# tabahi/WebSpeechAnalyzer

Measured on AMD Instinct MI355X. Metric: 53-feat frames/sec, higher is better.
Workload: dtype f32 front end / f64 tracker; 1 GPU; 1024 clips x 10 s @16 kHz mono per GPU, 1024-pt FFT, 25 ms hop, Segment Features (level 5); parallelism=1 GPU, batches_in_flight=6, streams=3

## Files before the change

webspeechanalyzer_amd/capi.py:

```python
import ctypes
import os
import subprocess

import numpy as np

_HERE = os.path.dirname(os.path.abspath(__file__))
NFEAT = 53


class WsaError(RuntimeError):
    pass


class _Config(ctypes.Structure):
    _fields_ = [("spec_type", ctypes.c_int32), ("output_level", ctypes.c_int32),
                ("f_min", ctypes.c_double), ("f_max", ctypes.c_double),
                ("N_fft_bins", ctypes.c_int32), ("N_mel_bins", ctypes.c_int32),
                ("window_width", ctypes.c_double), ("window_step", ctypes.c_double),
                ("pause_length", ctypes.c_double), ("min_seg_length", ctypes.c_double),
                ("auto_noise_gate", ctypes.c_int32),
                ("voiced_max_dB", ctypes.c_double), ("voiced_min_dB", ctypes.c_double),
                ("pre_norm_gain", ctypes.c_double), ("high_f_emph", ctypes.c_double)]


# ... 426 lines not shown
        return CHANNEL_MIX
    if isinstance(select, (bool, float)) or not 0 <= int(select) <= CHANNEL_MIX:
        raise WsaError(f"select {select!r}: a channel index or 'mix'")
    s = int(select)
    if channels is not None and s != CHANNEL_MIX and s >= int(channels):
        raise WsaError(f"select {s} is neither a channel below {int(channels)} nor 'mix'")
    return s


def pcm_decode(fmt, array, channels=1, select=0):
    f = pcm_format(fmt)
    ch = int(channels)
    if not 1 <= ch <= 64:
        raise WsaError(f"channel count {ch} outside 1 .. 64")
    sel = channel_select(select, ch)
    a = _pcm_array(fmt, f, array)
    size = a.size // _PCM_ELEMS.get(f, 1)
    last = ch - 1 if sel == CHANNEL_MIX else sel
    n = (size - 1 - last) // ch + 1 if size > last else 0
    out = np.zeros(n, np.float32)
    if lib().wsa_pcm_decode_select(f, a.ctypes.data, n, ch, sel, out.ctypes.data) != 0:
        raise WsaError("wsa_pcm_decode_select refused its arguments")
    return out


def pcm_channels_tile_frames(fmt, channels):
    return int(lib().wsa_pcm_channels_tile_frames(pcm_format(fmt), int(channels)))


def level_feature_count(output_level):
    return int(lib().wsa_level_feature_count(int(output_level)))


def rows_to_callbacks(level, step, meta, feat, payload):
    cbs = []
    if level in (4, 5):
        for m, f in zip(meta, feat):
            cbs.append([int(m[1]), [], [m[2] * step, (m[3] + 1) * step], payload(m, f)])
    elif level in (10, 12, 13):
        i = 0
        while i < len(meta):
            j = i
            while j < len(meta) and meta[j][1] == meta[i][1]:
                j += 1
            tm = [["%.3f" % (m[2] * step), "%.3f" % ((m[3] + 1) * step)] for m in meta[i:j]]
            rows_ = list(zip(meta[i:j], feat[i:j]))
            if level == 12:
                cut = next((q for q, (_, f) in enumerate(rows_) if f[23] != 0), len(rows_))
                rows_ = rows_[:cut]
            if level != 12 or rows_:
                cbs.append([int(meta[i][1]), [], tm, [payload(m, f) for m, f in rows_]])
            i = j
    return cbs


class Config(dict):

    def __init__(self, **kw):
        c = _Config()
        lib().wsa_config_default(ctypes.byref(c))
        super().__init__({k: getattr(c, k) for k, _ in _Config._fields_})
        for k, v in kw.items():
            if k not in self:
                raise KeyError(k)
            self[k] = v

    def c_struct(self):
        c = _Config()
        for k, t in _Config._fields_:
            setattr(c, k, int(self[k]) if t is ctypes.c_int32 else float(self[k]))
        return c


class Analyzer:

    def __init__(self, config=None, device=0):
        self.L = lib()
        self.config = config or Config()
        self.h = ctypes.c_void_p()
        cs = self.config.c_struct()
        st = self.L.wsa_create(ctypes.byref(cs), device, ctypes.byref(self.h))
        if st != 0:
            raise WsaError(f"wsa_create failed ({st}): {self.L.wsa_last_error(None).decode()}")
        self.device = device

    def _check(self, st):
        if st != 0:
            raise WsaError(f"libwsa error {st}: {self.L.wsa_last_error(self.h).decode()}")

    def geometry(self, fs):
        g = _Geometry()
        self._check(self.L.wsa_geometry_for(self.h, float(fs), ctypes.byref(g)))
        return {k: getattr(g, k) for k, _ in _Geometry._fields_}

    def bins_hz(self, fs):
        n = self.geometry(fs)["bands"]
        out = np.zeros(n)
        self._check(self.L.wsa_bins_hz(self.h, float(fs), out.ctypes.data, n))
        return out

    def batch(self, n_samples, fs, resample_to=None):
        return Batch(self, n_samples, fs, resample_to)

    def streams(self, n_streams, fs, frames_per_step=1, max_span_frames=1024, resample_to=None):
        return Streams(self, n_streams, fs, frames_per_step, max_span_frames, resample_to)

    def load_model(self, src):
        from . import nnmodel
        if isinstance(src, nnmodel.ModelSpec):
            spec = src
        elif isinstance(src, (tuple, list)):
            spec = nnmodel.parse(*src)
        else:
            spec = nnmodel.load_dir(src)
        return Model(self, spec)

    def trainer(self, spec, features, labels, n_val, batch_size, learning_rate):
        return Trainer(self, spec, features, labels, n_val, batch_size, learning_rate)

    def regress_trainer(self, spec, features, values, n_val, batch_size, learning_rate, out_min=None, out_max=None):
        return Trainer(self, spec, features, values, n_val, batch_size, learning_rate,
                       regression=(spec.out_min if out_min is None else out_min, spec.out_max if out_max is None else out_max))

    def train_group(self, trainers):
        return TrainGroup(self, trainers)

    def feature_db(self, features, durations, vocab_sizes=(), n_ord=0, first_row=0):
        return FeatureDBStats(self, features, durations, vocab_sizes, n_ord, first_row)

    def device_db(self, width, capacity):
        return FeatDB(self, width, capacity)

    def knn_store(self, width, n_classes, capacity):
        return KnnStore(self, width, n_classes, capacity)

    def ensemble(self, models):
        return Ensemble(self, models)

    def regress_group(self, models, ranges=None):
        return RegressGroup(self, models, ranges)

    def close(self):
        if self.h:
            self.L.wsa_destroy(self.h)
            self.h = ctypes.c_void_p()

    def __del__(self):
        try:
            self.close()
        except Exception:
            pass


class Batch:

    def __init__(self, an, n_samples, fs, resample_to=None):
        self.an, self.L = an, an.L
        self.n_samples = np.ascontiguousarray(n_samples, dtype=np.uint32)
        self.fs = float(fs) if np.ndim(fs) == 0 else None
        self.h = ctypes.c_void_p()
        if self.fs is None and not resample_to:
            raise WsaError("one rate per clip needs resample_to: a launch has one geometry")
        if resample_to and np.ndim(fs) > 0:
            self.n_samples_in, self.fs_in, self.fs = self.n_samples, np.ascontiguousarray(fs, dtype=np.float64), float(resample_to)
            if self.fs_in.shape != self.n_samples_in.shape:
                raise WsaError("fs as a sequence holds one rate per clip")
            an._check(self.L.wsa_batch_create_mixed(an.h, len(self.n_samples_in), self.n_samples_in.ctypes.data, self.fs_in.ctypes.data, self.fs, ctypes.byref(self.h)))
            self.n_samples = np.array([self.L.wsa_resample_length(int(n), float(f), self.fs) for n, f in zip(self.n_samples_in, self.fs_in)], np.uint32)
        elif resample_to:
            self.n_samples_in, self.fs_in, self.fs = self.n_samples, self.fs, float(resample_to)
            an._check(self.L.wsa_batch_create_resampled(an.h, len(self.n_samples_in), self.n_samples_in.ctypes.data, self.fs_in, self.fs, ctypes.byref(self.h)))
            self.n_samples = np.array([self.L.wsa_resample_length(int(n), self.fs_in, self.fs) for n in self.n_samples_in], np.uint32)
        else:
            an._check(self.L.wsa_batch_create(an.h, len(self.n_samples), self.n_samples.ctypes.data, self.fs, ctypes.byref(self.h)))
        info = _BatchInfo()
        an._check(self.L.wsa_batch_get_info(self.h, ctypes.byref(info)))
        self.info = {k: getattr(info, k) for k, _ in _BatchInfo._fields_}

    def run(self, d_pcm, clip_stride, stream=0):
        self.an._check(self.L.wsa_batch_run(self.h, d_pcm, int(clip_stride), stream))

    def run_frontend(self, d_pcm, clip_stride, stream=0):
        self.an._check(self.L.wsa_batch_run_frontend(self.h, d_pcm, int(clip_stride), stream))

    def run_backend(self, d_spectra, stream=0):
        self.an._check(self.L.wsa_batch_run_backend(self.h, d_spectra, stream))

    def converted_pcm(self, stream=0):
        stride = max(int(self.n_samples.max()) if len(self.n_samples) else 0, 1)
        out = np.zeros((len(self.n_samples), stride), np.float32)
        self.an._check(self.L.wsa_batch_copy_pcm(self.h, stream, out.ctypes.data, stride))
        return out

    def run_host(self, clips, stream=0):
        clips = [np.ascontiguousarray(c, dtype=np.float32) for c in clips]
        ptrs = (ctypes.c_void_p * len(clips))(*[c.ctypes.data for c in clips])
        self.an._check(self.L.wsa_batch_run_host(self.h, ptrs, stream))

    def run_host_i16(self, clips, channels=None, stream=0):
        clips = [np.ascontiguousarray(c, dtype=np.int16) for c in clips]
        ptrs = (ctypes.c_void_p * len(clips))(*[c.ctypes.data for c in clips])
        ch = None if channels is None else (ctypes.c_uint32 * len(clips))(*[int(c) for c in channels])
        self.an._check(self.L.wsa_batch_run_host_i16(self.h, ptrs, ch, stream))

    def _formats(self, formats, channels):
        n = len(self.n_samples)
        fm = [formats] * n if isinstance(formats, (str, int)) else list(formats)
        if len(fm) != n or (channels is not None and len(channels) != n):
            raise WsaError("one format (and one channel count) per clip")
        fm = (ctypes.c_int32 * max(n, 1))(*[pcm_format(f) if isinstance(f, str) else int(f) for f in fm])
        ch = None if channels is None else (ctypes.c_uint32 * max(n, 1))(*[int(c) for c in channels])
        return fm, ch

    def run_host_packed(self, clips, formats, channels=None, stream=0):
        fm, ch = self._formats(formats, channels)
        held = []
        ns_in = getattr(self, "n_samples_in", self.n_samples)
        for i, c in enumerate(clips):
            f = int(fm[i])
            a = _pcm_array(f, f, c) if f in _PCM_DTYPE else np.ascontiguousarray(c).reshape(-1)
            need = int(ns_in[i]) * (int(ch[i]) if ch is not None else 1) * _PCM_ELEMS.get(f, 1)
            if f in _PCM_DTYPE and a.size < need:
                raise WsaError(f"clip {i}: {a.size} elements, the plan's {int(ns_in[i])} frames need {need}")
            held.append(a)
        ptrs = (ctypes.c_void_p * max(len(held), 1))(*[a.ctypes.data for a in held])
        self.an._check(self.L.wsa_batch_run_host_packed(self.h, ptrs, fm, ch, stream))

    def set_input_format(self, formats, channels=None):
        fm, ch = self._formats(formats, channels)
        self.an._check(self.L.wsa_batch_set_input_format(self.h, fm, ch))

    def packed_offsets(self):
        return np.array([self.L.wsa_batch_packed_offset(self.h, i) for i in range(len(self.n_samples) + 1)], np.uint64)

    def run_packed(self, d_packed, stream=0):
        self.an._check(self.L.wsa_batch_run_packed(self.h, d_packed, stream))

    def _select_source(self, select, source):
        n = len(self.n_samples)
        sel = None
        if select is not None:
            sv = [select] * n if isinstance(select, (str, int)) else list(select)
            if len(sv) != n:
                raise WsaError("one select (a channel index or 'mix') per clip")
            sel = (ctypes.c_uint32 * max(n, 1))(*[channel_select(v) for v in sv])
        src = None
        if source is not None:
            if len(source) != n:
                raise WsaError("one source (a clip index) per clip")
            if any(int(v) < 0 or int(v) > 0xFFFFFFFF for v in source):
                raise WsaError("a source is a clip index")
            src = (ctypes.c_uint32 * max(n, 1))(*[int(v) for v in source])
        return sel, src

    def set_input_channels(self, formats, channels=None, select=None, source=None):
        fm, ch = self._formats(formats, channels)
        sel, src = self._select_source(select, source)
        self.an._check(self.L.wsa_batch_set_input_channels(self.h, fm, ch, sel, src))

    def run_host_channels(self, clips, formats, channels=None, select=None, source=None, stream=0):
        fm, ch = self._formats(formats, channels)
        sel, src = self._select_source(select, source)
        held, ptrs = [], []
        ns_in = getattr(self, "n_samples_in", self.n_samples)
        for i, c in enumerate(clips):
            if src is not None and int(src[i]) != i:
                ptrs.append(None)
                continue
            f = int(fm[i])
            a = _pcm_array(f, f, c) if f in _PCM_DTYPE else np.ascontiguousarray(c).reshape(-1)
            need = int(ns_in[i]) * (int(ch[i]) if ch is not None else 1) * _PCM_ELEMS.get(f, 1)
            if f in _PCM_DTYPE and a.size < need:
                raise WsaError(f"clip {i}: {a.size} elements, the plan's {int(ns_in[i])} frames need {need}")
            held.append(a)
            ptrs.append(a.ctypes.data)
        if len(ptrs) != len(self.n_samples):
            raise WsaError("one entry per clip (a consumer's may be None)")
        arr = (ctypes.c_void_p * max(len(ptrs), 1))(*ptrs)
        self.an._check(self.L.wsa_batch_run_host_channels(self.h, arr, fm, ch, sel, src, stream))

    def enable_timing(self, on):
        self.an._check(self.L.wsa_batch_enable_timing(self.h, int(on)))

    def keep_spectra(self, on=True):
        self.an._check(self.L.wsa_batch_keep_spectra(self.h, int(on)))
        return self

    def backend_reruns(self):
        n = ctypes.c_uint32(0)
        self.an._check(self.L.wsa_batch_backend_reruns(self.h, ctypes.byref(n)))
        return n.value

    def keep_counters(self, on=True):
        self.L.wsa_debug_batch_keep_counters.argtypes = [ctypes.c_void_p, ctypes.c_int32]
        self.an._check(self.L.wsa_debug_batch_keep_counters(self.h, int(on)))
        return self

    def tiers(self, stream=0):
        out = (ctypes.c_uint32 * 3)()
        self.L.wsa_debug_batch_tiers.argtypes = [ctypes.c_void_p, ctypes.c_void_p, ctypes.c_void_p]
        self.an._check(self.L.wsa_debug_batch_tiers(self.h, stream, out))
        return dict(flags=int(out[0]), spans=int(out[1]), redo=int(out[2]))

    def enable_trace(self, on=True):
        self.an._check(self.L.wsa_batch_enable_trace(self.h, int(on)))

    def trace(self, stream=0):
        n = self.info["n_frames_total"]
        out = np.zeros((n, 12))
        self.an._check(self.L.wsa_batch_copy_trace(self.h, stream, out.ctypes.data, max(n, 1)))
        return out

    def device_result(self, stream=0):
        r = _DeviceResult()
        self.an._check(self.L.wsa_batch_result(self.h, stream, ctypes.byref(r)))
        return r

    def stage_ms(self):
        out = np.zeros(4, np.float32)
        self.an._check(self.L.wsa_batch_stage_ms(self.h, out.ctypes.data))
        return out

    def rows(self, stream=0):
        r = self.device_result(stream)
        n, m, nc = r.n_rows, r.n_segments, r.n_clips
        meta = np.zeros((n, 8), np.int32)
        feat = np.zeros((n, NFEAT), np.float64)
        segs = np.zeros((m, 4), np.int32)
        roff = np.zeros(nc + 1, np.uint32)
        soff = np.zeros(nc + 1, np.uint32)
        self.an._check(self.L.wsa_batch_copy_rows(self.h, stream, meta.ctypes.data, feat.ctypes.data, max(n, 1),
                                                   segs.ctypes.data, max(m, 1), roff.ctypes.data, soff.ctypes.data))
        return dict(meta=meta, feat=feat, segments=segs, row_off=roff, seg_off=soff)

    def row_meta(self, stream=0):
        n = self.device_result(stream).n_rows
        meta = np.zeros((n, 8), np.int32)
        self.an._check(self.L.wsa_batch_copy_rows(self.h, stream, meta.ctypes.data, None, max(n, 1), None, 0, None, None))
        return meta

    def utterance_meta(self, stream=0):
        n = self.device_result(stream).n_utterance_rows
        meta = np.zeros((n, 4), np.int32)
        self.an._check(self.L.wsa_batch_copy_utterance(self.h, stream, meta.ctypes.data, None, max(n, 1), None))
        return meta

    def spectra(self, stream=0):
        words = self.info["n_frames_total"] * self.info["bands"]
        out = np.zeros((self.info["n_frames_total"], self.info["bands"]), np.uint32)
        foff = np.zeros(self.info["n_clips"] + 1, np.uint32)
        self.an._check(self.L.wsa_batch_copy_spectra(self.h, stream, out.ctypes.data, max(words, 1), foff.ctypes.data))
        return out, foff

    def formants(self, stream=0):
        n = self.info["n_frames_total"]
        out = np.zeros((n, 9), np.float32)
        self.an._check(self.L.wsa_batch_copy_formants(self.h, stream, out.ctypes.data, max(n, 1)))
        return out

    def utterance(self, stream=0):
        r = self.device_result(stream)
        n = r.n_utterance_rows
        meta = np.zeros((n, 4), np.int32)
        feat = np.zeros((n, 264), np.float64)
        off = np.zeros(len(self.n_samples) + 1, np.uint32)
        self.an._check(self.L.wsa_batch_copy_utterance(self.h, stream, meta.ctypes.data, feat.ctypes.data, max(n, 1), off.ctypes.data))
        return dict(meta=meta, feat=feat, off=off)

    def tracks(self, stream=0):
        class _TI(ctypes.Structure):
            _fields_ = [("n_segments", ctypes.c_uint32), ("n_points", ctypes.c_uint64), ("n_ranked", ctypes.c_uint64)]
        ti = _TI()
        self.an._check(self.L.wsa_batch_tracks_info(self.h, stream, ctypes.byref(ti)))
        seg_off = np.zeros((ti.n_segments + 1, 2), np.uint64)
        pts = np.zeros((max(int(ti.n_points), 1), 8), np.int32)
        rk = np.zeros(max(int(ti.n_ranked), 1), np.int32)
        self.an._check(self.L.wsa_batch_copy_tracks(self.h, stream, seg_off.ctypes.data, pts.ctypes.data, int(ti.n_points), rk.ctypes.data, int(ti.n_ranked)))
        return _track_records(seg_off, pts, rk, ti.n_segments)

    def callbacks(self, stream=0):
        r = self.rows(stream)
        level = int(self.an.config["output_level"])
        step = float(self.an.config["window_step"]) / 1e3
        utt = self.utterance(stream) if level == 11 else None
        trk = self.tracks(stream) if level == 3 else None
        fm = self.formants(stream) if level in (4, 10) else None
        foff = None
        if fm is not None:
            foff = np.zeros(len(self.n_samples) + 1, np.uint32)
            self.an._check(self.L.wsa_batch_copy_spectra(self.h, stream, None, 0, foff.ctypes.data))
        out = []
        for c in range(len(self.n_samples)):
            a, b = int(r["row_off"][c]), int(r["row_off"][c + 1])
            meta, feat = r["meta"][a:b], r["feat"][a:b]
            cbs = []
            payload = (lambda m, f: f[:23].copy() if level == 12 else f.copy()) if fm is None else (lambda m, f: fm[int(foff[c]) + m[6]: int(foff[c]) + m[6] + m[7]].copy())
            if level == 11:
                for k in range(int(utt["off"][c]), int(utt["off"][c + 1])):
                    m = utt["meta"][k]
                    cbs.append([0, [], [m[2] * step, (m[3] + 1) * step], utt["feat"][k].copy()])
            else:
                cbs = rows_to_callbacks(level, step, meta, feat, payload)
            sa, sb = int(r["seg_off"][c]), int(r["seg_off"][c + 1])
            if level == 3:
                cbs = [[k, [], trk[sa + k]] for k in range(sb - sa) if len(trk[sa + k]) > 0]
            out.append(dict(callbacks=cbs, segments_ci=[[int(s[1]), int(s[2])] for s in r["segments"][sa:sb]],
                            flags=[int(s[3]) for s in r["segments"][sa:sb]], meta=meta))
        return out

    def classify(self, model, stream=0):
        self.an._check(self.L.wsa_batch_classify(self.h, model.h, stream))
        self._model = model

    def class_result(self, stream=0):
        r = _ClassResult()
        self.an._check(self.L.wsa_batch_class_result(self.h, stream, ctypes.byref(r)))
        return r

    def classes(self, stream=0):
        r = self.class_result(stream)
        C, n, k = int(r.n_classes), int(r.n_rows), int(r.n_callbacks)
        prob, cb = np.zeros((n, C), np.float32), np.zeros((k, 4), np.int32)
        lab, conf = np.zeros(k, np.int32), np.zeros(k, np.float64)
        clip = np.zeros((int(r.n_clips), C), np.float64) if r.d_clip_conf else np.zeros((0, C))
        self.an._check(self.L.wsa_batch_copy_classes(self.h, stream, prob.ctypes.data, max(n, 1), cb.ctypes.data, lab.ctypes.data, conf.ctypes.data,
                                                      max(k, 1), clip.ctypes.data if r.d_clip_conf else None))
        return dict(prob=prob, cb=cb, cb_label=lab, cb_conf=conf, clip_conf=clip, labels=list(self._model.labels))

    def regress(self, model, out_min=None, out_max=None, stream=0):
        lo, hi = model.out_range(out_min, out_max)
        self.an._check(self.L.wsa_batch_regress(self.h, model.h, lo, hi, stream))
        self._model = model

    def values(self, stream=0):
        n = ctypes.c_uint32()
        self.an._check(self.L.wsa_batch_copy_values(self.h, stream, None, 0, ctypes.byref(n)))
        out = np.zeros(n.value, np.float64)
        self.an._check(self.L.wsa_batch_copy_values(self.h, stream, out.ctypes.data, max(n.value, 1), ctypes.byref(n)))
        return out

    def knn(self, store, k=10, stream=0):
        self.an._check(self.L.wsa_batch_knn(self.h, store.h, int(k), stream))
        self._knn = store

    def knn_result(self, stream=0):
        r = _KnnResult()
        self.an._check(self.L.wsa_batch_knn_result(self.h, stream, ctypes.byref(r)))
        return r

    def knn_classes(self, stream=0):
        r = self.knn_result(stream)
        n, C, k = int(r.n_rows), int(r.n_classes), int(r.k)
        out = dict(label=np.zeros(n, np.int32), conf=np.zeros((n, C), np.float64), nbr=np.zeros((n, k), np.int32), sim=np.zeros((n, k), np.float32), k_eff=int(r.k_eff))
        self.an._check(self.L.wsa_batch_copy_knn(self.h, stream, out["label"].ctypes.data, out["conf"].ctypes.data, out["nbr"].ctypes.data, out["sim"].ctypes.data, max(n, 1)))
        return out

    def knn_fold(self, stream=0):
        self.an._check(self.L.wsa_batch_knn_fold(self.h, stream))

    def knn_fold_classes(self, stream=0):
        r = _KnnFoldResult()
        self.an._check(self.L.wsa_batch_knn_fold_result(self.h, stream, ctypes.byref(r)))
        k, C = int(r.n_callbacks), int(r.n_classes)
        out = dict(cb=np.zeros((k, 4), np.int32), cb_label=np.zeros(k, np.int32), cb_conf=np.zeros(k, np.float64), clip_conf=np.zeros((int(r.n_clips), C), np.float64))
        self.an._check(self.L.wsa_batch_copy_knn_fold(self.h, stream, out["cb"].ctypes.data, out["cb_label"].ctypes.data, out["cb_conf"].ctypes.data, max(k, 1),
                                                       out["clip_conf"].ctypes.data))
        return out

    def regress_group(self, group, stream=0):
        self.an._check(self.L.wsa_batch_regress_group(self.h, group.h, stream))
        self._group = group

    def value_result(self, stream=0):
        r = _ValueResult()
        self.an._check(self.L.wsa_batch_value_result(self.h, stream, ctypes.byref(r)))
        return r

    def value_fold(self, stream=0):
        r = self.value_result(stream)
        H, n, k, nc = int(r.n_heads), int(r.n_rows), int(r.n_callbacks), int(r.n_clips)
        out = dict(value=np.zeros((H, n), np.float64))
        if r.d_cb:
            out.update(cb=np.zeros((k, 4), np.int32), cb_value=np.zeros((H, k)), cb_weight=np.zeros((H, k)),
                       clip_sum=np.zeros((H, nc)), clip_weight=np.zeros((H, nc)), clip_value=np.zeros((H, nc)))
        h = _ValueHost()
        h.rows_cap, h.cb_cap = max(n, 1), max(k, 1)
        for name, v in out.items():
            if name == "cb":
                h.cb = v.ctypes.data
            else:
                for d in range(H):
                    getattr(h, name)[d] = v[d].ctypes.data
        self.an._check(self.L.wsa_batch_copy_value_fold(self.h, stream, ctypes.byref(h)))
        return out

    def classify_ensemble(self, ensemble, stream=0):
        self.an._check(self.L.wsa_batch_classify_ensemble(self.h, ensemble.h, stream))
        self._ensemble = ensemble

    def ensemble_result(self, stream=0):
        r = _EnsembleResult()
        self.an._check(self.L.wsa_batch_ensemble_result(self.h, stream, ctypes.byref(r)))
        return r

    def ensemble_classes(self, stream=0):
        r = self.ensemble_result(stream)
        nm, n, k, nc = int(r.n_members), int(r.n_rows), int(r.n_callbacks), int(r.n_clips)
        fold = bool(r.d_cb)
        C = [int(r.n_classes[d]) for d in range(nm)]
        out = dict(prob=[np.zeros((n, c), np.float32) for c in C], labels=[list(m.labels) for m in self._ensemble.models])
        h = _EnsembleHost()
        h.rows_cap, h.cb_cap = max(n, 1), max(k, 1)
        if fold:
            for name, dt in (("cb_label", np.int32), ("cb_conf", np.float64), ("cb_all_max", np.float64)):
                out[name] = [np.zeros(k, dt) for _ in C]
            out["clip_conf"] = [np.zeros((nc, c), np.float64) for c in C]
            out.update(cb=np.zeros((k, 4), np.int32), cb_db=np.zeros(k, np.int32), cb_top_label=np.zeros(k, np.int32), cb_top_conf=np.zeros(k),
                       cb_min_db=np.zeros(k, np.int32), cb_entropy=np.zeros(k), clip_min_db=np.zeros(nc, np.int32))
        for name, v in out.items():
            if name == "labels":
                continue
            if isinstance(v, list):
                for d in range(nm):
                    getattr(h, name)[d] = v[d].ctypes.data
            else:
                setattr(h, name, v.ctypes.data)
        self.an._check(self.L.wsa_batch_copy_ensemble(self.h, stream, ctypes.byref(h)))
        return out

    def close(self):
        if self.h:
            self.L.wsa_batch_destroy(self.h)
            self.h = ctypes.c_void_p()

    def __del__(self):
        try:
            self.close()
        except Exception:
            pass


def _model_desc(spec):
    from . import nnmodel
    nl = len(spec.kernels)
    keep = [np.ascontiguousarray(k, np.float32) for k in spec.kernels] + [np.ascontiguousarray(b, np.float32) for b in spec.biases]
    units = (ctypes.c_int32 * (nl + 1))(*spec.units)
    acts = (ctypes.c_int32 * nl)(*[nnmodel.ACT[a] for a in spec.activations])
    kp = (ctypes.c_void_p * nl)(*[a.ctypes.data for a in keep[:nl]])
    bp = (ctypes.c_void_p * nl)(*[a.ctypes.data for a in keep[nl:]])
    mn, mx = np.ascontiguousarray(spec.in_min, np.float64), np.ascontiguousarray(spec.in_max, np.float64)
    labels = list(spec.labels)
    lab = (ctypes.c_char_p * len(labels))(*[str(x).encode() for x in labels]) if len(labels) == spec.n_classes else None
    d = _ModelDesc(nl, ctypes.cast(units, ctypes.c_void_p), ctypes.cast(acts, ctypes.c_void_p), ctypes.cast(kp, ctypes.c_void_p),
                   ctypes.cast(bp, ctypes.c_void_p), mn.ctypes.data, mx.ctypes.data, ctypes.cast(lab, ctypes.c_void_p) if lab is not None else None)
    return d, (keep, units, acts, kp, bp, mn, mx, lab)


class Model:

    def __init__(self, an, spec):
        self.an, self.L, self.spec = an, an.L, spec
        self.labels = list(spec.labels)
        self.n_classes = spec.n_classes
        self.n_inputs = int(spec.units[0])
        d, self._keep = _model_desc(spec)
        self.h = ctypes.c_void_p()
        an._check(self.L.wsa_model_create(an.h, ctypes.byref(d), ctypes.byref(self.h)))
        self._keep = None

    def classify_rows(self, d_feat, n_rows, d_prob, stream=0):
        self.an._check(self.L.wsa_classify_rows(self.h, d_feat, int(n_rows), d_prob, stream))

    def out_range(self, out_min=None, out_max=None):
        lo = getattr(self.spec, "out_min", None) if out_min is None else out_min
        hi = getattr(self.spec, "out_max", None) if out_max is None else out_max
        if lo is None or hi is None:
            raise ValueError("the model has no output range (out_min / out_max): not a regression model's spec, and none was given")
        return float(lo), float(hi)

    def regress_rows(self, d_feat, n_rows, d_value, out_min=None, out_max=None, stream=0):
        lo, hi = self.out_range(out_min, out_max)
        self.an._check(self.L.wsa_regress_rows(self.h, lo, hi, d_feat, int(n_rows), d_value, stream))

    def close(self):
        if self.h:
            self.L.wsa_model_destroy(self.h)
            self.h = ctypes.c_void_p()

    def __del__(self):
        try:
            self.close()
        except Exception:
            pass


class Trainer:

    def __init__(self, an, spec, features, labels, n_val, batch_size, learning_rate, regression=None, db=None):
        self.an, self.L, self.spec = an, an.L, spec
        self.out_range = None if regression is None else (float(regression[0]), float(regression[1]))
        lab = np.ascontiguousarray(labels, np.int32 if regression is None else np.float64)
        if db is not None:
            rows = np.ascontiguousarray(features, np.uint32)
            if rows.ndim != 1 or lab.shape != rows.shape:
                raise ValueError(f"rows {rows.shape} / labels {lab.shape}: expected [n] DB row indices and [n]")
            self.n_rows, self.n_val, self.n_train = rows.shape[0], int(n_val), rows.shape[0] - int(n_val)
# ... 1172 lines not shown
```

webspeechanalyzer_amd/csrc/api.hip:

```cpp
#include <cstdlib>
#include <map>
#include <mutex>
#include "host_plan.hpp"
#include "pcm_formats.hpp"

using namespace wsa;

thread_local std::string wsa_api::g_create_error;
using wsa_api::fail;

namespace wsa {
Tuning Tuning::from_env() {
    Tuning t;
    { const char* on = std::getenv("WSA_TUNING_ENV"); if (!on || on[0] != '1') return t; }
    auto num = [](const char* name, int dflt) { const char* e = std::getenv(name); return e && *e ? std::atoi(e) : dflt; };
    t.dbg = num("WSA_DBG", 0);
    t.no_pair = std::getenv("WSA_NO_PAIR") != nullptr; t.no_split = std::getenv("WSA_NO_SPLIT") != nullptr; t.no_quad = std::getenv("WSA_NO_QUAD") != nullptr; t.quad = std::getenv("WSA_QUAD") != nullptr; t.no_fuse = std::getenv("WSA_NO_FUSE") != nullptr;
    t.fe_fat = std::getenv("WSA_FE_FAT") != nullptr; t.peaks_lanes = std::getenv("WSA_PEAKS_LANES") != nullptr;
    t.full_table = num("WSA_FULL_TABLE", -1);
    t.tracker_wpc = num("WSA_TRACKER_WPC", 0); t.fin_wpc = num("WSA_FIN_WPC", 0); t.fpw = num("WSA_FPW", 0);
    t.fe_wg_per_cu = num("WSA_FE_WGS", 0); t.fe_no_queue = std::getenv("WSA_FE_NO_QUEUE") != nullptr; t.peaks_wpc = num("WSA_PEAKS_WPC", 0); t.peaks_w = num("WSA_PEAKS_W", 0); t.upload_threads = num("WSA_UPLOAD_THREADS", 0);
    t.rs_s = num("WSA_RS_S", 0); t.rs_j = num("WSA_RS_J", 0); t.rs_c = num("WSA_RS_C", 0); t.rs_one_launch = std::getenv("WSA_RS_ONE_LAUNCH") != nullptr;
    return t;
}
}

static std::mutex g_slab_mu;
static std::map<uintptr_t, size_t> g_slabs;
bool wsa_api::slab_of(const void* p, uintptr_t* base, size_t* size) {
    std::lock_guard<std::mutex> lk(g_slab_mu);
    auto it = g_slabs.upper_bound(reinterpret_cast<uintptr_t>(p));
    if (it == g_slabs.begin()) return false;
    --it;
    if (reinterpret_cast<uintptr_t>(p) >= it->first + it->second) return false;
    *base = it->first; *size = it->second;
    return true;
}

extern "C" {

int wsa_abi_version(void) { return WSA_ABI_VERSION; }

void wsa_config_default(wsa_config* c) {
    c->spec_type = 1; c->output_level = 4; c->f_min = 50; c->f_max = 4000; c->N_fft_bins = 256; c->N_mel_bins = 128;
    c->window_width = 25; c->window_step = 25; c->pause_length = 200; c->min_seg_length = 50; c->auto_noise_gate = 1;
    c->voiced_max_dB = 100; c->voiced_min_dB = 10; c->pre_norm_gain = 1000; c->high_f_emph = 0;
}

const char* wsa_last_error(const wsa_ctx* ctx) { return ctx ? ctx->err.c_str() : wsa_api::g_create_error.c_str(); }

wsa_status wsa_create(const wsa_config* cfg, int32_t device, wsa_ctx** out) {
    if (!cfg || !out) return fail(nullptr, WSA_ERR_INVALID, "null argument");
    *out = nullptr;
    int n = 0;
    if (hipGetDeviceCount(&n) != hipSuccess || n <= 0) return fail(nullptr, WSA_ERR_NO_DEVICE, "no HIP device visible (libwsa has no CPU path)");
    if (device < 0 || device >= n) return fail(nullptr, WSA_ERR_INVALID, "device ordinal out of range");
    hipDeviceProp_t prop;
    if (hipGetDeviceProperties(&prop, device) != hipSuccess) return fail(nullptr, WSA_ERR_NO_DEVICE, "hipGetDeviceProperties failed");
    if (std::strncmp(prop.gcnArchName, "gfx950", 6) != 0)
        return fail(nullptr, WSA_ERR_NO_DEVICE, std::string("libwsa is built for gfx950 only; device is ") + prop.gcnArchName);
    const int lv = cfg->output_level;
    if (!(lv == 1 || lv == 2 || lv == 3 || lv == 4 || lv == 5 || lv == 10 || lv == 11 || lv == 12 || lv == 13))
        return fail(nullptr, WSA_ERR_INVALID, "output_level must be 1, 2 (spectrum frames only), 3, 4, 5, 10, 11, 12 or 13");
    if (!(cfg->window_step > 0) || !(cfg->window_width > 0)) return fail(nullptr, WSA_ERR_INVALID, "window_width / window_step must be positive");
    wsa_ctx* c = new wsa_ctx();
    c->cfg = *cfg; c->device = device; c->n_cu = prop.multiProcessorCount;
    *out = c;
    return WSA_OK;
}

void wsa_destroy(wsa_ctx* ctx) { delete ctx; }

wsa_status wsa_geometry_for(const wsa_ctx* ctx, double fs, wsa_geometry* out) {
    if (!ctx || !out) return WSA_ERR_INVALID;
    FePlanHost p; std::string err;
    if (!build_fe_plan(ctx->cfg, fs, p, err)) return fail(const_cast<wsa_ctx*>(ctx), WSA_ERR_INVALID, err);
    out->nfft = p.nfft; out->win = p.win; out->hop = p.hop; out->bands = p.bands; out->kmax = p.kmax;
    return WSA_OK;
}

wsa_status wsa_bins_hz(const wsa_ctx* ctx, double fs, double* out, int32_t n) {
    if (!ctx || !out) return WSA_ERR_INVALID;
    FePlanHost p; std::string err;
    if (!build_fe_plan(ctx->cfg, fs, p, err)) return fail(const_cast<wsa_ctx*>(ctx), WSA_ERR_INVALID, err);
    if (n < p.bands) return fail(const_cast<wsa_ctx*>(ctx), WSA_ERR_INVALID, "bins_hz buffer too small");
    for (int i = 0; i < p.bands; i++) out[i] = p.bins_hz[i];
    return WSA_OK;
}

wsa_status wsa_host_alloc(wsa_ctx* ctx, uint64_t bytes, void** out) {
    if (!ctx || !out) return WSA_ERR_INVALID;
    *out = nullptr;
    HIP_TRY(ctx, hipSetDevice(ctx->device));
    HIP_TRY(ctx, hipHostMalloc(out, bytes ? (size_t)bytes : 1, hipHostMallocPortable));
    { std::lock_guard<std::mutex> lk(g_slab_mu); g_slabs[reinterpret_cast<uintptr_t>(*out)] = bytes ? (size_t)bytes : 1; }
    return WSA_OK;
}
void wsa_host_free(void* p) {
    if (!p) return;
    { std::lock_guard<std::mutex> lk(g_slab_mu); g_slabs.erase(reinterpret_cast<uintptr_t>(p)); }
    (void)hipHostFree(p);
}

wsa_status wsa_queue_create(wsa_ctx* ctx, void** stream) {
    if (!ctx || !stream) return WSA_ERR_INVALID;
    *stream = nullptr;
    HIP_TRY(ctx, hipSetDevice(ctx->device));
    hipStream_t s = nullptr;
    HIP_TRY(ctx, hipStreamCreateWithFlags(&s, hipStreamNonBlocking));
    *stream = s;
    return WSA_OK;
}
wsa_status wsa_queue_synchronize(wsa_ctx* ctx, void* stream) {
    if (!ctx) return WSA_ERR_INVALID;
    HIP_TRY(ctx, hipSetDevice(ctx->device));
    HIP_TRY(ctx, hipStreamSynchronize(reinterpret_cast<hipStream_t>(stream)));
    return WSA_OK;
}
void wsa_queue_destroy(wsa_ctx* ctx, void* stream) {
    if (!stream) return;
    if (ctx) (void)hipSetDevice(ctx->device);
    (void)hipStreamDestroy(reinterpret_cast<hipStream_t>(stream));
}

uint64_t wsa_resample_length(uint64_t n_in, double fs_in, double fs_out) { return fs_in > 0 && fs_out > 0 ? resample_length(n_in, fs_in, fs_out) : 0; }
uint64_t wsa_resample_ready(uint64_t n_in, double fs_in, double fs_out) { return fs_in > 0 && fs_out > 0 ? resample_ready(n_in, fs_in, fs_out) : 0; }

uint32_t wsa_pcm_channels_tile_frames(int32_t format, uint32_t channels) { return pcm_format_known(format) && channels >= 1 && channels <= 64 ? pcm_tile_frames(format, channels) : 0u; }

wsa_status wsa_pcm_decode_select(int32_t format, const void* in, uint64_t n_frames, uint32_t channels, uint32_t select, float* out) {
    if (channels < 1 || channels > 64 || (n_frames && (!in || !out)) || !pcm_format_known(format) || !pcm_select_known(select, channels)) return WSA_ERR_INVALID;
    const uint8_t* p = static_cast<const uint8_t*>(in);
    const uint32_t sb = pcm_sample_bytes(format);
    const uint64_t step = (uint64_t)channels * sb;
    for (uint64_t j = 0; j < n_frames; j++) {
        const uint8_t* fr = p + j * step;
        out[j] = select == WSA_CHANNEL_MIX ? pcm_mix_frame(channels, [&](uint32_t c) { return pcm_decode_bytes(format, fr + c * sb); }) : pcm_decode_bytes(format, fr + (uint64_t)select * sb);
    }
    return WSA_OK;
}

wsa_status wsa_pcm_decode(int32_t format, const void* in, uint64_t n_frames, uint32_t channels, float* out) {
    if (channels < 1 || channels > 64 || (n_frames && (!in || !out)) || !pcm_format_known(format)) return WSA_ERR_INVALID;
    const uint8_t* p = static_cast<const uint8_t*>(in);
    const uint64_t step = (uint64_t)channels * pcm_sample_bytes(format);
    for (uint64_t j = 0; j < n_frames; j++) out[j] = pcm_decode_bytes(format, p + j * step);
    return WSA_OK;
}

}
```

webspeechanalyzer_amd/csrc/batch_internal.hpp:

```cpp
#pragma once
#include "host_plan.hpp"
#include "pcm_formats.hpp"

struct wsa_batch {
    wsa_ctx* ctx = nullptr;
    uint32_t n_clips = 0;
    double fs = 0;
    std::vector<uint32_t> n_samples, n_frames, frame_off;
    uint32_t total_frames = 0, max_frames = 0, max_samples = 0;
    wsa::DevArena mem;
    wsa::FeDev fe;
    wsa::Derived D;
    wsa::BackEnd be;
    int n_waves = 0;
    uint32_t *d_n_frames = nullptr, *d_frame_off = nullptr, *d_spec = nullptr;
    uint2* d_order = nullptr;
    uint2* d_redo = nullptr;
    char* d_pool = nullptr; double* d_span_hdr = nullptr; bool split = false; size_t pool_bpf = 0;
    hipStream_t up_stream[8] = {}; hipEvent_t up_event[8] = {}, up_start = nullptr; bool up_ready = false;
    int16_t* d_i16 = nullptr; uint64_t i16_cap = 0; uint64_t* d_i16_off = nullptr; uint32_t *d_i16_ch = nullptr, *d_i16_ns = nullptr;
    std::vector<uint64_t> h_i16_off; std::vector<uint32_t> h_i16_ch;
    uint8_t* d_pk = nullptr; uint64_t pk_cap = 0; wsa::PcmClipDesc* d_pk_desc = nullptr; std::vector<wsa::PcmClipDesc> h_pk_desc;
    wsa::PcmClipDesc* d_pkf_desc = nullptr; std::vector<uint64_t> pkf_off; bool pkf_set = false;
    bool pkf_channels = false;
    bool pair = false;
    bool published = false;
    wsa::Tuning tune;
    uint32_t* d_span_hist = nullptr; uint2* d_span_key = nullptr;
    float* d_pcm_own = nullptr;
    bool rs_on = false; double fs_in = 0; std::vector<uint32_t> n_samples_in; uint32_t max_samples_in = 0;
    uint32_t *d_rs_n_in = nullptr, *d_rs_n_out = nullptr; float *d_rs_table = nullptr, *d_rs_pcm = nullptr; uint64_t rs_stride = 0;
    bool rs_mixed = false; wsa::RsMixedPlan rs_plan; wsa::RsClass* d_rs_cls = nullptr; uint32_t* d_rs_clip_class = nullptr; wsa::RsWork* d_rs_work = nullptr;
    bool keep_counters = false;
    bool counters_clean = false, end_clears = false, capturing = false, ever_captured = false;
    wsa::TrackGather trk;
    std::vector<int32_t> h_trk_seg; std::vector<uint32_t> h_seg_count;
    uint32_t res_utt = 0;
    double* d_trace = nullptr;
    uint32_t* h_totals = nullptr;
    uint32_t* h_totals_dev = nullptr;
    hipEvent_t ev[5] = {nullptr, nullptr, nullptr, nullptr, nullptr};
    bool timing = true, ran = false, full_table = false;
    uint32_t reruns = 0;
    uint32_t res_rows = 0, res_segs = 0, res_flags = 0;
    const uint32_t* spec_in_use = nullptr;
    wsa_cls* cls = nullptr;
    wsa_ecls* ecls = nullptr;
    int cls_last = 0;
    wsa_kcls* kcls = nullptr;
    wsa_rcls* rcls = nullptr;

    const std::vector<uint32_t>& host_samples() const { return rs_on ? n_samples_in : n_samples; }
    uint32_t max_host_samples() const { return rs_on ? max_samples_in : max_samples; }
    uint64_t staging_stride() const { return (max_host_samples() + 3u) & ~3ull; }
};

namespace wsa_api {
#pragma GCC visibility push(hidden)
wsa_status run_impl(wsa_batch* b, const float* d_pcm, uint64_t stride, const uint32_t* d_spec_in, bool fe, bool be, hipStream_t s);
wsa_status fetch_totals(wsa_batch* b, hipStream_t s);
inline wsa_status no_run_yet(wsa_batch* b) { return fail(b->ctx, WSA_ERR_INVALID, "no run on this batch yet"); }
#pragma GCC visibility pop
}
```

webspeechanalyzer_amd/csrc/batch_run.hip:

```cpp
#include <algorithm>
#include "batch_internal.hpp"

using namespace wsa;
using wsa_api::fail;

namespace wsa {
__global__ void batch_publish_kernel(const uint32_t* totals, const uint32_t* counters, uint32_t* host) {
    if (threadIdx.x == 0) {
        host[0] = totals[0]; host[1] = totals[1]; host[2] = counters[1]; host[3] = totals[3];
        __threadfence_system();
    }
}
__global__ void batch_clear_kernel(uint32_t* counters, uint32_t* totals, uint32_t* span_hist) {
    if (threadIdx.x < 16) counters[threadIdx.x] = 0;
    if (threadIdx.x < 4) totals[threadIdx.x] = 0;
    if (span_hist) for (int b = threadIdx.x; b < SPAN_BUCKETS; b += blockDim.x) span_hist[b] = 0;
}
}

static wsa_status run_backend_stages(wsa_batch* b, const uint32_t* d_spec, bool skip_peaks, hipStream_t s) {
    wsa_ctx* ctx = b->ctx;
    const Derived& D = b->D;
    const BackEnd& B = b->be;
    b->published = false;
    if (D.level <= 2) return WSA_OK;
    const int dbg = b->tune.dbg;
    uint32_t* counters = B.d_counters + 4;
    PkParams pk; pk.spec = d_spec; pk.rec = B.rec; pk.total_frames = b->total_frames; pk.bands = b->fe.plan.bands;
    pk.flags = B.d_counters + 1; pk.dbg = (b->tune.dbg >> DBG_PEAKS_SHIFT) & 0xff; pk.lanes_only = b->tune.peaks_lanes ? 1 : 0;
    pk.wpc = b->tune.peaks_wpc; pk.round_bins = b->tune.peaks_w;
    if (!skip_peaks) launch_peaks(pk, s);
    GateParams g;
    B.fill(g, D);
    g.n_frames = b->d_n_frames; g.frame_off = b->d_frame_off; g.trace = b->d_trace; g.dbg = dbg; g.prio = 1;
    const bool ordered = !(dbg & DBG_UNSORTED_SPANS);
    g.span_hist = ordered ? b->d_span_hist : nullptr; g.span_key = b->d_span_key;
    launch_gate(g, s);
    TrParams t;
    B.fill(t, D);
    t.frame_off = b->d_frame_off; t.trace = b->d_trace; t.dbg = dbg;
    t.order = ordered ? b->d_order : nullptr; t.redo = b->d_redo; t.redo_count = counters + 2;
    t.fin_waves = b->tune.fin_wpc >= 1 && b->tune.fin_wpc <= 32 ? ctx->n_cu * b->tune.fin_wpc : 0;
    t.quad = b->split && !b->tune.no_quad && (b->tune.quad || b->total_frames >= 1200000u) ? 1 : 0;
    t.quad_waves = (int)std::min<size_t>((size_t)b->n_waves, ((size_t)b->n_clips * (size_t)B.seg_cap + 3) / 4 + 1);
    t.pool = b->split ? b->d_pool : nullptr; t.pool_bpf = (uint32_t)b->pool_bpf; t.span_hdr = b->split ? b->d_span_hdr : nullptr;
    if (t.order) launch_span_order(t, b->d_span_hist, b->d_span_key, b->d_order, counters, s);
    if (b->timing) HIP_TRY(ctx, hipEventRecord(b->ev[2], s));
    launch_tracker(t, b->n_waves, b->full_table, b->pair, s);
    if (b->timing) HIP_TRY(ctx, hipEventRecord(b->ev[3], s));
    CompactParams cp;
    B.fill(cp, D);
    cp.clip_rows = B.d_clip_rows; cp.flags = B.d_counters + 1; cp.fused = b->tune.no_fuse ? 0 : 1;
    cp.host = D.tail_kernel ? nullptr : b->h_totals_dev;
    b->published = compact_is_fused(cp) && cp.host != nullptr;
    const bool self_clear = b->published && !b->capturing && !b->keep_counters;
    cp.clr_counters = self_clear ? B.d_counters : nullptr; cp.clr_hist = self_clear ? b->d_span_hist : nullptr;
    b->end_clears = self_clear;
    launch_compact(cp, s);
    if (D.level == 11) {
        UttParams u;
        B.fill(u, b->d_frame_off);
        launch_utterance(u, s);
    }
    if (D.level == 12) {
        CoefParams q;
        B.fill(q, b->d_frame_off);
        q.total_frames = b->total_frames;
        launch_coeffs(q, b->n_clips * (uint32_t)B.row_cap, s);
    }
    HIP_TRY(ctx, hipGetLastError());
    return WSA_OK;
}

wsa_status wsa_api::run_impl(wsa_batch* b, const float* d_pcm, uint64_t stride, const uint32_t* d_spec_in, bool fe, bool be, hipStream_t s) {
    wsa_ctx* ctx = b->ctx;
    HIP_TRY(ctx, hipSetDevice(ctx->device));
    {
        hipStreamCaptureStatus cap = hipStreamCaptureStatusNone;
        if (s && hipStreamIsCapturing(s, &cap) != hipSuccess) { (void)hipGetLastError(); cap = hipStreamCaptureStatusNone; }
        b->capturing = cap != hipStreamCaptureStatusNone;
        if (b->capturing) b->ever_captured = true;
    }
    if (!b->counters_clean || b->ever_captured) hipLaunchKernelGGL(batch_clear_kernel, dim3(1), dim3(256), 0, s, b->be.d_counters, b->be.d_totals, b->d_span_hist);
    b->counters_clean = false; b->end_clears = false;
    if (b->timing) HIP_TRY(ctx, hipEventRecord(b->ev[0], s));
    const uint32_t* spec = d_spec_in ? d_spec_in : b->d_spec;
    if (fe) {
        if (!d_pcm && b->total_frames) return fail(ctx, WSA_ERR_INVALID, "null PCM pointer");
        if (stride < b->max_host_samples() && b->n_clips > 1) return fail(ctx, WSA_ERR_INVALID, "clip_stride smaller than the longest clip");
        if (b->rs_mixed) {
            RsMixedParams r; r.in = d_pcm; r.stride_in = stride; r.out = b->d_rs_pcm; r.stride_out = b->rs_stride; r.n_in = b->d_rs_n_in; r.n_out = b->d_rs_n_out;
            r.tables = b->d_rs_table; r.cls = b->d_rs_cls; r.clip_class = b->d_rs_clip_class; r.work = b->d_rs_work;
            launch_resample_mixed(r, b->rs_plan, !b->tune.rs_one_launch, s);
            HIP_TRY(ctx, hipGetLastError());
            d_pcm = b->d_rs_pcm; stride = b->rs_stride;
        } else if (b->rs_on) {
            RsParams r; r.in = d_pcm; r.stride_in = stride; r.out = b->d_rs_pcm; r.stride_out = b->rs_stride;
            r.n_in = b->d_rs_n_in; r.n_out = b->d_rs_n_out; r.table = b->d_rs_table; r.ratio = b->fs_in / b->fs; r.S = b->tune.rs_s > 0 ? b->tune.rs_s : resample_stride(b->fs_in, b->fs);
            r.J = b->tune.rs_j > 0 ? b->tune.rs_j : resample_outputs_per_lane(r.S, r.ratio); r.span = resample_span(r.ratio, r.S, r.J); r.chunks = b->tune.rs_c > 0 ? b->tune.rs_c : 1;
            launch_resample(r, b->n_clips, b->max_samples, s);
            HIP_TRY(ctx, hipGetLastError());
            d_pcm = b->d_rs_pcm; stride = b->rs_stride;
        }
        FeParams p;
        b->fe.fill(p, b->tune.fe_fat);
        p.pcm = d_pcm; p.clip_stride = stride; p.n_frames = b->d_n_frames; p.frame_off = b->d_frame_off; p.spec = b->d_spec;
        p.frames_per_wave = b->tune.fpw > 0 ? b->tune.fpw : 25; p.wg_per_cu = b->tune.fe_wg_per_cu;
        p.queue = b->tune.fe_no_queue ? nullptr : b->be.d_counters + 8; p.n_cu = b->ctx->n_cu;
        launch_frontend(p, (int)b->n_clips, (int)b->max_frames, b->fe.plan.R, b->fe.plan.three, s);
        HIP_TRY(ctx, hipGetLastError());
    }
    if (b->timing) HIP_TRY(ctx, hipEventRecord(b->ev[1], s));
    if (be) {
        if (const wsa_status st = run_backend_stages(b, spec, false, s); st != WSA_OK) return st;
    } else if (b->timing) { HIP_TRY(ctx, hipEventRecord(b->ev[2], s)); HIP_TRY(ctx, hipEventRecord(b->ev[3], s)); }
    if (!(be && b->published)) hipLaunchKernelGGL(batch_publish_kernel, dim3(1), dim3(64), 0, s, b->be.d_totals, b->be.d_counters, b->h_totals_dev);
    if (b->timing) HIP_TRY(ctx, hipEventRecord(b->ev[4], s));
    b->ran = true; b->spec_in_use = spec;
    b->counters_clean = be && b->end_clears && !b->capturing;
    return WSA_OK;
}

wsa_status wsa_api::fetch_totals(wsa_batch* b, hipStream_t s) {
    wsa_ctx* ctx = b->ctx;
    if (!b->ran) return no_run_yet(b);
    HIP_TRY(ctx, hipSetDevice(ctx->device));
    HIP_TRY(ctx, hipStreamSynchronize(s));
    const volatile uint32_t* ht = b->h_totals;
    b->res_rows = ht[0]; b->res_segs = ht[1]; b->res_flags = ht[2]; b->res_utt = ht[3];
    if (b->res_flags & 2u) {
        b->full_table = true; b->reruns++;
        hipLaunchKernelGGL(batch_clear_kernel, dim3(1), dim3(256), 0, s, b->be.d_counters, b->be.d_totals, b->d_span_hist);
        const bool tm = b->timing; b->timing = false;
        const wsa_status st = run_backend_stages(b, b->spec_in_use, true, s);
        b->timing = tm;
        if (st != WSA_OK) return st;
        if (!b->published) hipLaunchKernelGGL(batch_publish_kernel, dim3(1), dim3(64), 0, s, b->be.d_totals, b->be.d_counters, b->h_totals_dev);
        HIP_TRY(ctx, hipStreamSynchronize(s));
        b->res_rows = ht[0]; b->res_segs = ht[1]; b->res_flags = ht[2]; b->res_utt = ht[3];
    }
    if (b->res_flags & 1u) return fail(ctx, WSA_ERR_CAPACITY, "a device-side arena overflowed; results are invalid");
    return WSA_OK;
}

extern "C" {

wsa_status wsa_batch_run(wsa_batch* b, const float* d_pcm, uint64_t clip_stride, void* stream) {
    if (!b) return WSA_ERR_INVALID;
    return wsa_api::run_impl(b, d_pcm, clip_stride, nullptr, true, true, reinterpret_cast<hipStream_t>(stream));
}
wsa_status wsa_batch_run_frontend(wsa_batch* b, const float* d_pcm, uint64_t clip_stride, void* stream) {
    if (!b) return WSA_ERR_INVALID;
    return wsa_api::run_impl(b, d_pcm, clip_stride, nullptr, true, false, reinterpret_cast<hipStream_t>(stream));
}
wsa_status wsa_batch_run_backend(wsa_batch* b, const uint32_t* d_spectra, void* stream) {
    if (!b || !d_spectra) return WSA_ERR_INVALID;
    return wsa_api::run_impl(b, nullptr, 0, d_spectra, false, true, reinterpret_cast<hipStream_t>(stream));
}

void wsa_batch_view_internal(wsa_batch* b, wsa_batch_view* v) {
    v->ctx = b->ctx; v->level = b->ctx->cfg.output_level; v->n_clips = b->n_clips; v->rows_cap = b->n_clips * (uint32_t)b->be.row_cap;
    v->d_utt_feat = b->be.d_utt_feat; v->d_utt_off = b->be.d_utt_off; v->utt_cap = b->n_clips * (uint32_t)b->be.seg_cap;
    v->d_meta = b->be.d_meta; v->d_feat = b->be.d_feat; v->d_row_off = b->be.d_row_off; v->reruns = b->reruns; v->cls = &b->cls; v->ecls = &b->ecls; v->cls_last = &b->cls_last; v->kcls = &b->kcls; v->rcls = &b->rcls;
}
wsa_status wsa_batch_fetch_internal(wsa_batch* b, hipStream_t s) { return wsa_api::fetch_totals(b, s); }
const uint32_t* wsa_batch_counters_internal(wsa_batch* b, int keep, wsa_ctx** ctx) {
    if (keep >= 0) b->keep_counters = keep != 0;
    if (ctx) *ctx = b->ctx;
    return b->be.d_counters;
}

wsa_ctx* wsa_batch_ctx_internal(const wsa_batch* b) { return b ? b->ctx : nullptr; }

int wsa_debug_batch_counters(wsa_batch* b, uint32_t* out16) {
    if (!b || !out16) return WSA_ERR_INVALID;
    return hipMemcpy(out16, b->be.d_counters, 16 * sizeof(uint32_t), hipMemcpyDeviceToHost) == hipSuccess ? WSA_OK : WSA_ERR_HIP;
}

}
```

webspeechanalyzer_amd/csrc/tracker.hip:

```cpp
#include <type_traits>
#include "wsa_internal.hpp"
#include "jsmath_device.hpp"
#include "wave_ops.hpp"
#include "tracker_score.hpp"
#include "tracker_features.hpp"

#ifdef WSA_TUNING
#define WSA_TUNE(bits_) (p.dbg & (bits_))
#else
#define WSA_TUNE(bits_) false
#endif

namespace wsa {

constexpr int MAXC = 64;
constexpr int AC_MAX = 320;
constexpr int PAIR_AC = 64;
constexpr int PAIR_GSZ = 4384;
constexpr int QUAD_AC = 38;
constexpr int QUAD_GSZ = 2496;
constexpr int AC_FAST = 140;

struct Ws {
    int32_t *tr_len, *tr_slot, *tr_rank;
    double *tr_sumE, *tr_sumEbin;
    int4* pt;
    int4* ptx;
    int32_t* pt_key;
    int32_t *d_p0, *d_p1, *d_gen;
    float *fr, *sm1;
    double *dB, *Aev;
    int32_t *q_idx, *sorted; double* q_mb;
};

__host__ __device__ inline size_t align16(size_t x) { return (x + 15) & ~(size_t)15; }

__host__ __device__ __forceinline__ Ws carve_ws(char* base, int T, int P, int F, int PX, size_t* bytes) {
    Ws w;
    size_t o = 0;
#define WSA_CARVE(field, type, count) do { w.field = reinterpret_cast<type*>(base + o); \
        o = align16(o + sizeof(type) * (size_t)(count)); } while (0)
    WSA_CARVE(tr_len, int32_t, T); WSA_CARVE(tr_slot, int32_t, T); WSA_CARVE(tr_rank, int32_t, T);
    WSA_CARVE(tr_sumE, double, T); WSA_CARVE(tr_sumEbin, double, T);
    WSA_CARVE(pt, int4, P); WSA_CARVE(ptx, int4, PX); WSA_CARVE(pt_key, int32_t, P);
    WSA_CARVE(d_p0, int32_t, F + 2); WSA_CARVE(d_p1, int32_t, F + 2); WSA_CARVE(d_gen, int32_t, F + 2);
    WSA_CARVE(fr, float, (size_t)(F + 2) * 9); WSA_CARVE(sm1, float, F + 2);
    WSA_CARVE(dB, double, (size_t)3 * (F + 2)); WSA_CARVE(Aev, double, (size_t)3 * (F + 2));
    WSA_CARVE(q_idx, int32_t, T); WSA_CARVE(sorted, int32_t, T); WSA_CARVE(q_mb, double, T);
#undef WSA_CARVE
    if (bytes) *bytes = o;
    return w;
}

constexpr int GW_MAX = 32;
static_assert(GW_MAX <= MAXC, "a frame's new tracks / points (one per lane of its span's group) fit the MAXC per frame that tracker_pool_bpf gives a span region");
size_t tracker_pool_bpf() { size_t b = 0; (void)carve_ws(nullptr, MAXC, MAXC, 1, 0, &b); return align16(b) + 256; }
size_t tracker_ws_bytes(int tcap, int pcap, int fcap, bool raw_tracks) { size_t b = 0; (void)carve_ws(nullptr, tcap, pcap, fcap, raw_tracks ? pcap : 0, &b); return align16(b) + 256; }
struct PhaseClock {
    unsigned long long cy[5] = {0, 0, 0, 0, 0}, t0 = 0;
    __device__ __forceinline__ void start(bool on) { if (on) t0 = __builtin_readcyclecounter(); }
    __device__ __forceinline__ void lap(bool on, int k) { if (on) { const unsigned long long now = __builtin_readcyclecounter(); cy[k] += now - t0; t0 = now; } }
};

struct SpanState {
    uint32_t clip; int my_seg; int32_t* sg; uint32_t foff;
    int start, len, c_ci; uint32_t f_begin, f_end; double ctx_max, floor_;
    int n_tr, n_pt, n_act, stale_d, stale_p1, gen;
    double accG, accL;
    bool overflow, act_overflow;
    Ws W; int aev_stride;
    unsigned long long ph[4]; PhaseClock acp;
    __device__ __forceinline__ void clear_tracks() { n_tr = n_pt = n_act = 0; stale_d = -1; stale_p1 = 0; accG = accL = 0; }
    __device__ __forceinline__ void begin(const TrParams& p, uint32_t clip_, int seg_) {
        clip = clip_; my_seg = seg_; foff = p.frame_off[clip];
        start = len = c_ci = 0; f_begin = f_end = 0; ctx_max = floor_ = 0;
        clear_tracks(); overflow = act_overflow = false;
        ph[0] = ph[1] = ph[2] = ph[3] = 0; acp = PhaseClock();
    }
    __device__ __forceinline__ void load_segment(const TrParams& p, bool frames) {
        sg = p.seg_i + ((uint64_t)clip * p.seg_cap + my_seg) * 8;
        start = sg[SEG_START]; len = sg[SEG_LEN]; c_ci = sg[SEG_CCI];
        if (frames) { f_begin = (uint32_t)sg[SEG_FBEGIN]; f_end = (uint32_t)sg[SEG_FEND]; }
        ctx_max = p.seg_d[((uint64_t)clip * p.seg_cap + my_seg) * 2];
        floor_ = p.seg_d[((uint64_t)clip * p.seg_cap + my_seg) * 2 + 1];
    }
    __device__ __forceinline__ void totals(double& S, double& C) const { C = wave_sum_f64(accL); S = accG - C; }
};

template <int AC, bool QUAD = false>
struct OneLds {
    static constexpr int SCRATCH = MAXC * (4 + 4 + 8 + 8) + 64 * 8 + MAXC * 8 + MAXC * 4;
    static constexpr int LDS_ONE = AC * 52 + SCRATCH;
    static constexpr int BYTES = (QUAD && 4 * QUAD_GSZ > LDS_ONE) ? 4 * QUAD_GSZ : LDS_ONE;
    static_assert((AC * 52) % 16 == 0, "the scratch arrays start 16-byte aligned");
    static constexpr int FRCAP = (AC * 52 - AC * 16) / 40;
    static_assert(FRCAP <= FEAT_LDS_MAX, "finalize_generic hands formant_features_lds every span that fits the block");
    unsigned char* big;
    double *s_plo, *s_phi;
    unsigned long long* s_best; uint32_t *s_pk, *s_amp;
    int32_t *s_pr_j, *s_pr_o, *s_asg;
    double *a_vel, *a_sumE, *a_sumEbin;
    unsigned long long* a_mmask;
    int32_t *a_last_frame, *a_len, *a_gid;
    uint32_t *a_bins, *a_amp;
    double* f_qmb; int32_t *f_qidx, *f_sorted; float *f_fr, *f_sm;
    __device__ __forceinline__ explicit OneLds(unsigned char* b) : big(b) {
        a_vel = reinterpret_cast<double*>(big); a_sumE = a_vel + AC; a_sumEbin = a_sumE + AC;
        a_mmask = reinterpret_cast<unsigned long long*>(a_sumEbin + AC);
        a_last_frame = reinterpret_cast<int32_t*>(a_mmask + AC); a_len = a_last_frame + AC; a_gid = a_len + AC;
        a_bins = reinterpret_cast<uint32_t*>(a_gid + AC); a_amp = a_bins + AC;
        f_qmb = reinterpret_cast<double*>(big); f_qidx = reinterpret_cast<int32_t*>(f_qmb + AC); f_sorted = f_qidx + AC;
        f_fr = reinterpret_cast<float*>(f_sorted + AC); f_sm = f_fr + FRCAP * 9;
        s_plo = reinterpret_cast<double*>(big + AC * 52); s_phi = s_plo + MAXC;
        s_best = reinterpret_cast<unsigned long long*>(s_phi + MAXC);
        s_pk = reinterpret_cast<uint32_t*>(s_best + MAXC); s_amp = s_pk + MAXC;
        s_pr_j = reinterpret_cast<int32_t*>(s_amp + MAXC); s_pr_o = s_pr_j + 64; s_asg = s_pr_o + 64;
    }
};
template <int AC, bool QUAD = false>
__device__ __forceinline__ OneLds<AC, QUAD> carve_lds() {
    __shared__ __attribute__((aligned(16))) unsigned char s_big[OneLds<AC, QUAD>::BYTES];
    return OneLds<AC, QUAD>(s_big);
}

struct SpanTurn { uint32_t item, clip = 0, seg = 0, total = 0; uint64_t group = 0; };
enum { DEAL_SPANS, DEAL_GROUPS, DEAL_FINALIZE };  enum { SPAN_DONE, SPAN_SKIP, SPAN_TAKE };
template <int DEAL, int NGR = 1>
__device__ __forceinline__ int next_span(const TrParams& p, SpanTurn& t) {
    if (DEAL == DEAL_FINALIZE) {
        const uint32_t total = p.counters[p.order_cnt];
        const uint64_t idx = (uint64_t)t.item * gridDim.x + blockIdx.x;
        if (idx >= total) return SPAN_DONE;
        t.item++;
        const uint2 e = p.order[idx];
        t.clip = e.x; t.seg = e.y;
    }
    else if (DEAL == DEAL_GROUPS) {
        t.total = p.counters[p.order_cnt];
        const uint32_t npairs = (t.total + (uint32_t)NGR - 1u) / (uint32_t)NGR, W_ = gridDim.x, r = t.item;
        if ((uint64_t)r * W_ >= npairs) return SPAN_DONE;
        t.item++;
        t.group = (uint64_t)r * W_ + ((r & 1u) ? W_ - 1u - blockIdx.x : blockIdx.x);
        if (t.group >= npairs) return SPAN_SKIP;
    }
    else if (p.order) {
        const uint32_t total = p.counters[p.order_cnt], W_ = gridDim.x, r = t.item;
        if ((uint64_t)r * W_ >= total) return SPAN_DONE;
        t.item++;
        const uint64_t idx = (uint64_t)r * W_ + ((r & 1u) ? W_ - 1u - blockIdx.x : blockIdx.x);
        if (idx >= total) return SPAN_SKIP;
        const uint2 e = p.order[idx];
        t.clip = e.x; t.seg = e.y;
    } else {
        t.seg = t.item / p.n_clips; t.clip = t.item - t.seg * p.n_clips;
        if (t.seg >= p.counters[0]) return SPAN_DONE;
        t.item += gridDim.x;
        if (t.seg >= p.seg_count[t.clip]) return SPAN_SKIP;
    }
    return SPAN_TAKE;
}

}
#include "tracker_finalize.hpp"
#include "tracker_one.hpp"
#include "tracker_group.hpp"
namespace wsa {

template <int AC, bool RAW>
__device__ __forceinline__ void one_span_body(const TrParams& p) {
    const OneLds<AC> L = carve_lds<AC>();
    const int lane = threadIdx.x;
    SpanState sp;
    sp.W = carve_ws(p.ws + (uint64_t)blockIdx.x * p.ws_stride, p.tcap, p.pcap, p.fcap, RAW ? p.pcap : 0, nullptr);
    sp.gen = 0; sp.aev_stride = p.fcap + 2;
    for (int d = lane; d < p.fcap + 2; d += 64) sp.W.d_gen[d] = 0;
    wsync();
    SpanTurn t{p.order ? 0u : blockIdx.x};
    for (;;) {
        const int turn = next_span<DEAL_SPANS>(p, t);
        if (turn == SPAN_DONE) break;
        if (turn == SPAN_SKIP) continue;
        sp.begin(p, t.clip, (int)t.seg); sp.load_segment(p, true); sp.gen++;
        const unsigned long long tk0 = (WSA_TUNE(DBG_CYCLES)) ? __builtin_readcyclecounter() : 0ull;
        track_span<AC, RAW>(p, sp, L, lane);
        const unsigned long long tk1 = (WSA_TUNE(DBG_CYCLES)) ? __builtin_readcyclecounter() : 0ull;
        finish_span<AC, RAW, false>(p, sp, L, lane);
        trace_span_cycles(p, sp, lane, tk0, tk1);
        if (sp.overflow && lane == 0) atomicOr(&p.shared[1], sp.act_overflow && AC < AC_MAX ? 2u : 1u);
        wsync();
    }
}
template <int AC, bool RAW>
__device__ __forceinline__ void stream_body(const TrParams& p) {
    const OneLds<AC> L = carve_lds<AC>();
    const int lane = threadIdx.x;
    SpanState sp;
    sp.W = carve_ws(p.ws + (uint64_t)blockIdx.x * p.ws_stride, p.tcap, p.pcap, p.fcap, RAW ? p.pcap : 0, nullptr);
    sp.aev_stride = p.fcap + 2;
    wsync();
    sp.begin(p, blockIdx.x, 0);
    const unsigned long long tk0 = (WSA_TUNE(DBG_CYCLES)) ? __builtin_readcyclecounter() : 0ull;
    track_stream<AC, RAW>(p, sp, L, lane);
    trace_span_cycles(p, sp, lane, tk0, tk0);
    if (sp.overflow && lane == 0) atomicOr(&p.shared[1], 1u);
    wsync();
}
template <int AC, int GW, int SPLIT>
__device__ __forceinline__ void group_body(const TrParams& p) {
    const OneLds<AC, GW == 16> L = carve_lds<AC, GW == 16>();
    const int lane = threadIdx.x;
    SpanState sp;
    sp.gen = 0; sp.aev_stride = p.fcap + 2;
    if (!SPLIT) for (int h = 0; h < 2; h++) {
        const Ws Wh = carve_ws(p.ws + ((uint64_t)blockIdx.x * 2 + h) * p.ws_stride, p.tcap, p.pcap, p.fcap, 0, nullptr);
        for (int d = lane; d < p.fcap + 2; d += 64) Wh.d_gen[d] = 0;
    }
    wsync();
    SpanTurn t{p.order ? 0u : blockIdx.x};
    for (;;) {
        const int turn = next_span<DEAL_GROUPS, 64 / GW>(p, t);
        if (turn == SPAN_DONE) break;
        if (turn == SPAN_SKIP) continue;
        sp.gen++;
        track_group<AC, GW, SPLIT>(p, sp, L, lane, t);
    }
}
template <int AC>
__device__ __forceinline__ void finalize_body(const TrParams& p) {
    const OneLds<AC> L = carve_lds<AC>();
    const int lane = threadIdx.x;
    SpanState sp;
    wsync();
    SpanTurn t{p.order ? 0u : blockIdx.x};
    for (;;) {
        if (next_span<DEAL_FINALIZE>(p, t) == SPAN_DONE) break;
        sp.begin(p, t.clip, (int)t.seg); sp.load_segment(p, true);
        finalize_from_header<AC>(p, sp, L, lane);
    }
}

__global__ __launch_bounds__(64) __attribute__((amdgpu_waves_per_eu(4, 4))) void tracker_kernel_fast(TrParams p) { one_span_body<AC_FAST, false>(p); }
__global__ __launch_bounds__(64) __attribute__((amdgpu_waves_per_eu(3, 4))) void tracker_kernel_pair(TrParams p) {
    __builtin_amdgcn_s_setprio(3);
    group_body<AC_FAST, 32, 0>(p);
}
__global__ __launch_bounds__(64) __attribute__((amdgpu_waves_per_eu(4, 4))) void tracker_kernel_pair_acc(TrParams p) {
    __builtin_amdgcn_s_setprio(3);
    group_body<AC_FAST, 32, 1>(p);
}
__global__ __launch_bounds__(64) __attribute__((amdgpu_waves_per_eu(4, 4))) void tracker_kernel_quad_acc(TrParams p) {
    __builtin_amdgcn_s_setprio(3);
    group_body<AC_FAST, 16, 1>(p);
}
__global__ __launch_bounds__(64) __attribute__((amdgpu_waves_per_eu(4, 4))) void tracker_kernel_finalize(TrParams p) {
    __builtin_amdgcn_s_setprio(3);
    finalize_body<AC_FAST>(p);
}
__global__ __launch_bounds__(64) void tracker_kernel_full(TrParams p) { one_span_body<AC_MAX, false>(p); }
__global__ __launch_bounds__(64) void tracker_kernel_raw(TrParams p) { one_span_body<AC_MAX, true>(p); }
__global__ __launch_bounds__(64) void tracker_kernel_stream(TrParams p) { stream_body<AC_MAX, false>(p); }
__global__ __launch_bounds__(64) void tracker_kernel_stream_raw(TrParams p) { stream_body<AC_MAX, true>(p); }

constexpr int ORDER_T = 256;
__global__ __launch_bounds__(ORDER_T) void span_order_kernel(const uint32_t* hist, const uint2* key, const uint32_t* seg_count, uint32_t n_clips, int seg_cap, uint2* order, uint32_t* counters) {
    __shared__ uint32_t offs[SPAN_BUCKETS], part[ORDER_T];
    const int tid = threadIdx.x;
    constexpr int PER = SPAN_BUCKETS / ORDER_T;
    uint32_t mine[PER], sum = 0;
#pragma unroll
    for (int q = 0; q < PER; q++) { mine[q] = hist[tid * PER + q]; sum += mine[q]; }
    part[tid] = sum;
    __syncthreads();
    for (int d = 1; d < ORDER_T; d <<= 1) {
        const uint32_t add = tid >= d ? part[tid - d] : 0u;
        __syncthreads();
        part[tid] += add;
        __syncthreads();
    }
    uint32_t run = part[tid] - sum;
#pragma unroll
    for (int q = 0; q < PER; q++) { offs[tid * PER + q] = run; run += mine[q]; }
    if (blockIdx.x == 0 && tid == ORDER_T - 1) counters[1] = part[tid];
    __syncthreads();
    const uint32_t clip = blockIdx.x * ORDER_T + tid;
    if (clip >= n_clips) return;
    const uint32_t ns = seg_count[clip];
    for (uint32_t k = 0; k < ns; k++) {
        const uint2 e = key[(uint64_t)clip * seg_cap + k];
        order[offs[e.x] + e.y] = make_uint2(clip, k);
    }
}

void launch_span_order(const TrParams& p, uint32_t* span_hist, const uint2* span_key, uint2* order, uint32_t* counters, hipStream_t s) {
    if (p.n_clips == 0) return;
    hipLaunchKernelGGL(span_order_kernel, dim3((p.n_clips + ORDER_T - 1) / ORDER_T), dim3(ORDER_T), 0, s, span_hist, span_key, p.seg_count, p.n_clips, p.seg_cap, order, counters);
}

void launch_tracker_stream(const TrParams& p, uint32_t n_streams, hipStream_t s) {
    if (n_streams == 0) return;
    static_assert(AC_MAX == TR_ACT_MAX, "the streams' saved active table is sized for the full variant");
    if (p.level == 3) hipLaunchKernelGGL(tracker_kernel_stream_raw, dim3(n_streams), dim3(64), 0, s, p);
    else hipLaunchKernelGGL(tracker_kernel_stream, dim3(n_streams), dim3(64), 0, s, p);
}

void launch_tracker(const TrParams& p, int n_waves, bool full_table, bool pair, hipStream_t s) {
    if (n_waves <= 0) return;
    if (p.level == 3) hipLaunchKernelGGL(tracker_kernel_raw, dim3(n_waves), dim3(64), 0, s, p);
    else if (full_table) hipLaunchKernelGGL(tracker_kernel_full, dim3(n_waves), dim3(64), 0, s, p);
    else if (pair && p.order && p.redo && (!p.trace || (p.dbg & DBG_CYCLES))) {
        if (p.pool && p.span_hdr) {
            if (p.quad) hipLaunchKernelGGL(tracker_kernel_quad_acc, dim3(p.quad_waves > 0 ? p.quad_waves : n_waves), dim3(64), 0, s, p);
            else hipLaunchKernelGGL(tracker_kernel_pair_acc, dim3(n_waves), dim3(64), 0, s, p);
            hipLaunchKernelGGL(tracker_kernel_finalize, dim3(p.fin_waves > 0 ? p.fin_waves : 2 * n_waves), dim3(64), 0, s, p);
        }
        else hipLaunchKernelGGL(tracker_kernel_pair, dim3(n_waves), dim3(64), 0, s, p);
        TrParams r = p; r.order = p.redo; r.order_cnt = 2; r.pool = nullptr; r.span_hdr = nullptr;
        const int redo_waves = p.quad ? 1024 : 128;
        hipLaunchKernelGGL(tracker_kernel_fast, dim3(n_waves < redo_waves ? n_waves : redo_waves), dim3(64), 0, s, r);
    }
    else hipLaunchKernelGGL(tracker_kernel_fast, dim3(n_waves), dim3(64), 0, s, p);
}

__global__ void compact_count_kernel(CompactParams p) {
    const uint32_t c = blockIdx.x * blockDim.x + threadIdx.x;
    if (c >= p.n_clips) return;
    const uint32_t ns = p.seg_count[c];
    const int32_t* sg = p.seg_i + (uint64_t)c * p.seg_cap * 8;
    uint32_t r = 0;
    for (uint32_t k = 0; k < ns; k++) if (sg[8 * k + SEG_FLAG] >= 0) r += (uint32_t)sg[8 * k + SEG_NROWS];
    p.clip_row_off[c] = r;
}
constexpr int CSCAN_T = 1024;
template <bool COUNT>
__global__ __launch_bounds__(CSCAN_T) void compact_scan_kernel(CompactParams p) {
    __shared__ uint32_t s_rows[CSCAN_T], s_segs[CSCAN_T];
    const int tid = threadIdx.x;
    const uint32_t per = (p.n_clips + CSCAN_T - 1) / CSCAN_T;
    const uint32_t c0 = min(p.n_clips, tid * per), c1 = min(p.n_clips, c0 + per);
    uint32_t rs = 0, ss = 0;
    for (uint32_t c = c0; c < c1; c++) {
        if (COUNT) {
            const uint32_t ns = p.seg_count[c];
            const int32_t* sg = p.seg_i + (uint64_t)c * p.seg_cap * 8;
            uint32_t r = 0;
            for (uint32_t k = 0; k < ns; k++) if (sg[8 * k + SEG_FLAG] >= 0) r += (uint32_t)sg[8 * k + SEG_NROWS];
            p.clip_row_off[c] = r;
        }
        ss += p.seg_count[c]; rs += p.clip_row_off[c];
    }
    s_rows[tid] = rs; s_segs[tid] = ss;
    __syncthreads();
    for (int d = 1; d < CSCAN_T; d <<= 1) {
        const uint32_t ar_ = tid >= d ? s_rows[tid - d] : 0u, as_ = tid >= d ? s_segs[tid - d] : 0u;
        __syncthreads();
        s_rows[tid] += ar_; s_segs[tid] += as_;
        __syncthreads();
    }
    if (tid == CSCAN_T - 1) {
        p.totals[0] = s_rows[tid]; p.totals[1] = s_segs[tid];
        p.clip_row_off[p.n_clips] = s_rows[tid]; p.clip_seg_off[p.n_clips] = s_segs[tid];
    }
    uint32_t ar = s_rows[tid] - rs, as = s_segs[tid] - ss;
    for (uint32_t c = c0; c < c1; c++) {
        const uint32_t r = p.clip_row_off[c];
        p.clip_row_off[c] = ar; p.clip_seg_off[c] = as; as += p.seg_count[c]; ar += r;
    }
}

template <bool FUSED>
__global__ __launch_bounds__(64) void compact_gather_kernel(CompactParams p) {
    const uint32_t clip = blockIdx.x;
    const int lane = threadIdx.x;
    const uint32_t nseg = p.seg_count[clip];
    if (FUSED) {
        uint32_t rs = 0, ss = 0;
        for (uint32_t i = lane; i < clip; i += 64) { rs += p.clip_rows[i]; ss += p.seg_count[i]; }
        rs = wave_sum_u32(rs); ss = wave_sum_u32(ss);
        if (lane == 0) { p.clip_row_off[clip] = rs; p.clip_seg_off[clip] = ss; }
        if (clip == 0) {
            uint32_t rt = 0, st = 0;
            for (uint32_t i = lane; i < p.n_clips; i += 64) { rt += p.clip_rows[i]; st += p.seg_count[i]; }
            rt = wave_sum_u32(rt); st = wave_sum_u32(st);
            if (lane == 0) {
                p.totals[0] = rt; p.totals[1] = st; p.clip_row_off[p.n_clips] = rt; p.clip_seg_off[p.n_clips] = st;
                if (p.host) { p.host[0] = rt; p.host[1] = st; p.host[2] = p.flags[0]; p.host[3] = p.totals[3]; __threadfence_system(); }
            }
            if (p.clr_counters) {
                wsync();
                if (lane < 16) p.clr_counters[lane] = 0u;
                if (lane < 4) p.totals[lane] = 0u;
                if (p.clr_hist) for (int b = lane; b < SPAN_BUCKETS; b += 64) p.clr_hist[b] = 0u;
            }
        }
        wsync();
    }
    const uint32_t so = p.clip_seg_off[clip];
    const int32_t* sg = p.seg_i + (uint64_t)clip * p.seg_cap * 8;
    for (uint32_t i = lane; i < nseg; i += 64) {
        int32_t* o = p.seg_out + (uint64_t)(so + i) * 4;
        o[0] = (int32_t)clip; o[1] = sg[8 * i + SEG_START]; o[2] = sg[8 * i + SEG_LEN]; o[3] = sg[8 * i + SEG_FLAG];
    }
    uint32_t ro = p.clip_row_off[clip];
    int si = 0;
    int32_t* cy = p.carry ? p.carry + (uint64_t)clip * CARRY_WORDS : nullptr;
    const int seg_before = cy ? cy[0] : 0, res_before = cy ? cy[1] : 0;
    bool lost = false;
    for (uint32_t k = 0; k < nseg; k++) {
        const int flag = sg[8 * k + SEG_FLAG];
        if (flag < 0) continue;
        const int nr = sg[8 * k + SEG_NROWS];
        const uint32_t r0 = (uint32_t)sg[8 * k + SEG_ROW0];
        const int gsi = res_before + si;
        int32_t ts, tl;
        if (gsi >= seg_before) { ts = sg[8 * (gsi - seg_before) + SEG_START]; tl = sg[8 * (gsi - seg_before) + SEG_LEN]; }
        else {
            if (seg_before - gsi > CARRY_HIST) lost = true;
            ts = cy[2 + 2 * (gsi % CARRY_HIST)]; tl = cy[3 + 2 * (gsi % CARRY_HIST)];
        }
        for (int i = lane; i < nr; i += 64) {
            const int32_t* m = p.row_meta_in + (uint64_t)(r0 + i) * 8;
            int32_t* o = p.row_meta_out + (uint64_t)(ro + i) * 8;
            o[0] = m[0]; o[1] = gsi; o[4] = seg_before + m[4]; o[5] = m[5]; o[6] = m[6]; o[7] = m[7];
            if (p.level == 10 || p.level == 13) { o[2] = ts + m[2]; o[3] = m[3]; }
            else { o[2] = ts; o[3] = tl; }
        }
        for (int i = lane; i < nr * WSA_NFEAT; i += 64) p.row_feat_out[(uint64_t)ro * WSA_NFEAT + i] = p.row_feat_in[(uint64_t)r0 * WSA_NFEAT + i];
        ro += (uint32_t)nr;
        si++;
    }
    if (cy) {
        wsync();
        if (lane == 0) {
            for (uint32_t k = 0; k < nseg; k++) {
                const int g = seg_before + (int)k;
                cy[2 + 2 * (g % CARRY_HIST)] = sg[8 * k + SEG_START]; cy[3 + 2 * (g % CARRY_HIST)] = sg[8 * k + SEG_LEN];
            }
            cy[0] = seg_before + (int)nseg; cy[1] = res_before + si;
            if (lost) atomicOr(&p.totals[2], 1u);
        }
    }
}

int compact_path(const CompactParams& p) {
    if (p.n_clips == 0) return COMPACT_NOTHING;
    if (p.fused && !p.carry && p.clip_rows && p.n_clips <= 4096) return COMPACT_FUSED;
    return p.n_clips <= 2 * CSCAN_T ? COMPACT_SCAN : COMPACT_COUNT_SCAN;
}
void launch_compact(const CompactParams& p, hipStream_t s) {
    const int path = compact_path(p);
    if (path == COMPACT_NOTHING) return;
    if (path == COMPACT_FUSED) { hipLaunchKernelGGL(compact_gather_kernel<true>, dim3(p.n_clips), dim3(64), 0, s, p); return; }
    if (path == COMPACT_SCAN) hipLaunchKernelGGL(compact_scan_kernel<true>, dim3(1), dim3(CSCAN_T), 0, s, p);
    else {
        hipLaunchKernelGGL(compact_count_kernel, dim3((p.n_clips + 255) / 256), dim3(256), 0, s, p);
        hipLaunchKernelGGL(compact_scan_kernel<false>, dim3(1), dim3(CSCAN_T), 0, s, p);
    }
    hipLaunchKernelGGL(compact_gather_kernel<false>, dim3(p.n_clips), dim3(64), 0, s, p);
}
bool compact_is_fused(const CompactParams& p) { return compact_path(p) == COMPACT_FUSED; }

}
```

webspeechanalyzer_amd/csrc/tracker_finalize.hpp:

```cpp
#pragma once

namespace wsa {

__device__ __forceinline__ long long take_rows(const TrParams& p, SpanState& sp, int lane, int n) {
    uint32_t r0 = 0;
    if (lane == 0) r0 = atomicAdd(&p.clip_rows[sp.clip], (uint32_t)n);
    r0 = (uint32_t)read_lane_i32((int)r0, 0);
    if ((uint64_t)r0 + (uint32_t)n > p.row_cap) { sp.overflow = true; return -1; }
    return (long long)sp.clip * p.row_cap + r0;
}
template <typename Clear>
__device__ __forceinline__ int qualify_tracks(const Ws& W, int n_tr, int lane, double* qmb, int32_t* qt, Clear&& clear) {
    int nq = 0;
    for (int base = 0; base < n_tr; base += 64) {
        const int t = base + lane;
        bool q = false; double mb = 0;
        if (t < n_tr) {
            clear(t);
            const int tl = W.tr_len[t]; const double sb = W.tr_sumEbin[t], se = W.tr_sumE[t];
            if (tl >= 2) { mb = sb / se; q = mb >= 7; }
        }
        const uint64_t mask = __ballot(q);
        if (q) { const int pos = nq + __popcll(mask & lanemask_lt(lane)); qmb[pos] = mb; qt[pos] = t; }
        nq += __popcll(mask);
    }
    return nq;
}
template <typename Put>
__device__ __forceinline__ void rank_tracks(int nq, const double* qmb, int lane, Put&& put) {
    for (int base = 0; base < nq; base += 64) {
        const int qi = base + lane;
        if (qi < nq) {
            const double mb = qmb[qi];
            int rank = 0;
            for (int u = 0; u < nq; u++) { const double o = qmb[u]; rank += (o < mb || (o == mb && u < qi)) ? 1 : 0; }
            put(rank, qi);
        }
    }
}
template <typename Key>
__device__ __forceinline__ int assign_slots(int nq, const double* qmb, const int32_t* qt, const int32_t* srt, int lane, Key&& key) {
    int n_part = 0;
    double last = 0; int slot = 0; bool stopped = false;
    for (int base = 0; base < nq && !stopped; base += 64) {
        const int r = base + lane;
        double mb = 0; int t = 0;
        if (r < nq) { const int qi = srt[r]; mb = qmb[qi]; t = qt[qi]; }
        uint64_t todo = __ballot(r < nq);
        int myslot = -1;
        while (todo) {
            const uint64_t jm = __ballot(((todo >> lane) & 1ull) && fabs(mb - last) > 20);
            if (jm == 0ull) { if ((todo >> lane) & 1ull) myslot = slot; break; }
            const int j = __ffsll((long long)jm) - 1;
            if (((todo >> lane) & 1ull) && lane < j) myslot = slot;
            last = read_lane_f64(mb, j);
            slot++;
            if (slot >= 3) { stopped = true; break; }
            todo &= ~lanemask_lt(j);
        }
        if (myslot >= 0) key(t, (r << 2) | myslot);
        n_part += __popcll(__ballot(myslot >= 0));
    }
    return n_part;
}
template <typename Part>
__device__ __forceinline__ bool files_past_the_end(const SpanState& sp, int lane, bool by_index, Part&& takes_part) {
    bool bad = false;
    for (int base = sp.len; base <= (by_index ? sp.c_ci + 1 : -1); base += 64) {
        const int d = base + lane;
        if (d <= sp.c_ci + 1 && sp.W.d_gen[d] == sp.gen)
            for (int q = sp.W.d_p0[d]; q < sp.W.d_p1[d]; q++) if (takes_part(q)) bad = true;
    }
    if (sp.stale_d >= sp.len && lane == 0)
        for (int q = 0; q < sp.stale_p1; q++) if (takes_part(q)) bad = true;
    return bad;
}
template <typename Key, typename KeyOf, typename Point>
__device__ __forceinline__ void straighten_select(const TrParams& p, const SpanState& sp, int lane, float* fr, float* smv, KeyOf&& key_of, Point&& point) {
    for (int base = 0; base < ((WSA_TUNE(DBG_NO_STRAIGHTEN)) ? 0 : sp.len); base += 64) {
        const int d = base + lane;
        if (d < sp.len) {
            float f9[9];
#pragma unroll
            for (int q = 0; q < 9; q++) f9[q] = 0.f;
            float sm = 0.f;
            const int a1 = (sp.stale_d == d) ? sp.stale_p1 : 0;
            const int dg = sp.W.d_gen[d], dp0 = sp.W.d_p0[d], dp1 = sp.W.d_p1[d];
            const bool has_main = dg == sp.gen;
            const int b0 = has_main ? dp0 : 0, b1 = has_main ? dp1 : 0;
            Key last_key = -1;
            for (;;) {
                Key best_key = sizeof(Key) == 4 ? (Key)0x7fffffff : (Key)0x7fffffffffffffffLL; int best_q = -1;
                for (int part = 0; part < 2; part++) {
                    const int q0 = part ? b0 : 0, q1 = part ? b1 : a1;
                    for (int q = q0; q < q1; q++) {
                        const Key key = key_of(q);
                        if (key > last_key && key < best_key) { best_key = key; best_q = q; }
                    }
                }
                if (best_q < 0) break;
                last_key = best_key;
                int l; double f, wd, E;
                point(best_q, l, f, wd, E);
                const float cur = l == 0 ? f9[0] : (l == 1 ? f9[3] : f9[6]);
                if ((double)cur > sp.floor_ && (double)cur < f && l < 2) l++;
                const float ff = (float)f, Ef = (float)E, wf = (float)wd;
                if (l == 0) { f9[0] = ff; f9[1] = Ef; f9[2] = wf; }
                else if (l == 1) { f9[3] = ff; f9[4] = Ef; f9[5] = wf; }
                else { f9[6] = ff; f9[7] = Ef; f9[8] = wf; }
                sm = (float)((double)sm + E);
            }
#pragma unroll
            for (int q = 0; q < 9; q++) fr[9 * d + q] = f9[q];
            smv[d] = sm;
        }
    }
}
template <bool LANES, typename Feat>
__device__ __forceinline__ void write_rows(const TrParams& p, SpanState& sp, int lane, const float* fr, const float* smv, Feat&& features) {
    if (p.formants && (p.level == 4 || p.level == 10)) {
        for (int q = lane; q < 9 * sp.len; q += 64) { const int d = q / 9; p.formants[((uint64_t)sp.foff + (((uint32_t)sp.start + (uint32_t)d) & p.ring_mask)) * 9 + (uint32_t)(q - 9 * d)] = fr[q]; }
        if (p.sums) { for (int q = lane; q < sp.len; q += 64) p.sums[(uint64_t)sp.foff + (((uint32_t)sp.start + (uint32_t)q) & p.ring_mask)] = smv[q]; }
    }
    double accS, accC; sp.totals(accS, accC);
    const double cs = accC / accS;
    const double lg_ctx = jsm::log10(sp.ctx_max);
    if (p.level == 4 || p.level == 5) {
        const long long r0 = take_rows(p, sp, lane, 1);
        if (r0 < 0) return;
        double* x = p.row_feat + (uint64_t)r0 * WSA_NFEAT;
        if (WSA_TUNE(DBG_CYCLES)) sp.ph[2] = __builtin_readcyclecounter();
        if (p.level == 5) {
            if (!(WSA_TUNE(DBG_NO_FEATURES))) features(fr, sp.len, x);
            if (WSA_TUNE(DBG_CYCLES)) sp.ph[3] = __builtin_readcyclecounter();
            if (lane == 0) { x[0] = sp.len; x[1] = sqrt((double)sp.len); x[2] = cs; x[3] = lg_ctx; x[4] = sp.floor_; }
        } else if (lane < WSA_NFEAT) x[lane] = 0;
        if (lane == 0) {
            int32_t* m = p.row_meta + (uint64_t)r0 * 8;
            m[0] = (int32_t)sp.clip; m[1] = 0; m[2] = 0; m[3] = 0; m[4] = sp.my_seg; m[5] = 0; m[6] = sp.start; m[7] = sp.len;
            sp.sg[SEG_FLAG] = 1; sp.sg[SEG_NROWS] = 1; sp.sg[SEG_ROW0] = (int32_t)r0;
        }
        return;
    }
    int nsyl = 0, my_si = 0, my_sl = 0;
    {
        int si = -1, cc = 0, uu = 0;
        for (int base = 0; base < sp.len; base += 64) {
            const int dd = base + lane;
            const float smq = dd < sp.len ? smv[dd] : 0.f;
            const int lim = min(64, sp.len - base);
            for (int j = 0; j < lim; j++) {
                const int e2 = base + j;
                const double v = __builtin_bit_cast(float, read_lane_i32(__builtin_bit_cast(int, smq), j));
                if (v > sp.floor_) { cc = 0; uu++; if (si < 0) si = e2; } else cc++;
                if ((uu > 20 && cc > 0) || (uu > 10 && cc > 1) || (uu > 0 && cc > 4) || (e2 >= sp.len - 1 && uu > 4)) {
                    const int t = e2 - cc;
                    if (t - si > 1) {
                        if (LANES && nsyl < 64) { if (lane == nsyl) { my_si = si; my_sl = t - si; } }
                        else if (lane == 0) { sp.W.q_idx[2 * nsyl] = si; sp.W.q_idx[2 * nsyl + 1] = t - si; }
                        nsyl++;
                        si = -1; uu = 0;
                    }
                }
            }
        }
    }
    wsync();
    long long r0 = 0;
    if (nsyl > 0) { r0 = take_rows(p, sp, lane, nsyl); if (r0 < 0) return; }
    for (int k = 0; k < nsyl; k++) {
        const int si = LANES && k < 64 ? read_lane_i32(my_si, k) : sp.W.q_idx[2 * k], sl = LANES && k < 64 ? read_lane_i32(my_sl, k) : sp.W.q_idx[2 * k + 1];
        double* x = p.row_feat + (uint64_t)(r0 + k) * WSA_NFEAT;
        if (p.level == 13) {
            if (!(WSA_TUNE(DBG_NO_FEATURES))) features(fr + 9 * si, sl, x);
            if (lane == 0) { x[0] = sl; x[1] = sqrt((double)sl); x[2] = cs; x[3] = lg_ctx; x[4] = sp.floor_; }
        } else if (lane < WSA_NFEAT) x[lane] = 0;
        if (lane == 0) {
            int32_t* m = p.row_meta + (uint64_t)(r0 + k) * 8;
            m[0] = (int32_t)sp.clip; m[1] = 0; m[2] = si; m[3] = sl; m[4] = sp.my_seg; m[5] = k; m[6] = sp.start + si; m[7] = sl;
        }
    }
    if (lane == 0) { sp.sg[SEG_FLAG] = nsyl > 0 ? 1 : 0; sp.sg[SEG_NROWS] = nsyl; sp.sg[SEG_ROW0] = (int32_t)r0; }
}
template <int AC, bool G>
__device__ __forceinline__ bool finalize_lds(const TrParams& p, SpanState& sp, const OneLds<AC>& L, int lane) {
    constexpr int BIG = OneLds<AC>::BYTES;
    const int off_u = (int)align16((size_t)2 * sp.n_tr);
    const int rank_bytes = 16 * sp.n_tr, fr_bytes = G ? 0 : (int)align16((size_t)40 * sp.len);
    const int off_pt = off_u + fr_bytes;
    const bool pe_lds = !G && off_pt + 12 * sp.n_pt <= BIG;
    const int ppb = pe_lds ? 12 : 4;
    if (sp.n_tr > 8000 || sp.n_pt > 60000 || off_u + rank_bytes > BIG || off_pt + ppb * sp.n_pt > BIG || off_pt + FEAT_SCRATCH * 8 > BIG) return false;
    int16_t* const trk_key = reinterpret_cast<int16_t*>(L.big);
    double* const qmb = reinterpret_cast<double*>(L.big + off_u);
    int32_t* const qt = reinterpret_cast<int32_t*>(L.big + off_u + 8 * sp.n_tr);
    int32_t* const srt = qt + sp.n_tr;
    float* const fr = G ? sp.W.fr : reinterpret_cast<float*>(L.big + off_u);
    float* const smv = G ? sp.W.sm1 : fr + 9 * sp.len;
    double* const pE = reinterpret_cast<double*>(L.big + off_pt);
    uint32_t* const pkb = reinterpret_cast<uint32_t*>(L.big + off_pt + (pe_lds ? 8 * sp.n_pt : 0));
    auto energy_of = [&](int q) __attribute__((always_inline)) -> double { return pe_lds ? pE[q] : reinterpret_cast<const double*>(sp.W.pt + q)[1]; };
    if (WSA_TUNE(DBG_CYCLES)) sp.ph[0] = sp.ph[1] = sp.ph[2] = sp.ph[3] = __builtin_readcyclecounter();
    const int nq = qualify_tracks(sp.W, sp.n_tr, lane, qmb, qt, [&](int t) __attribute__((always_inline)) { trk_key[t] = -1; });
    wsync();
    rank_tracks(nq, qmb, lane, [&](int rank, int qi) __attribute__((always_inline)) { srt[rank] = qi; });
    wsync();
    const int n_part = assign_slots(nq, qmb, qt, srt, lane, [&](int t, int key) __attribute__((always_inline)) { trk_key[t] = (int16_t)key; });
    wsync();
    const int off_tbl = (int)align16((size_t)off_pt + (size_t)ppb * (size_t)sp.n_pt);
    const int tbl_bytes = 4 * (sp.len + 1) + 2 * (sp.len + 1) * n_part;
    const bool use_tbl = !G && n_part <= 32 && sp.c_ci + 1 < 0x7fff && sp.stale_d < 0x7fff && off_tbl + tbl_bytes <= BIG && !(p.dbg & DBG_SELECT_LOOP);
    uint32_t* const tblm = reinterpret_cast<uint32_t*>(L.big + off_tbl);
    uint16_t* const tbl = reinterpret_cast<uint16_t*>(tblm + sp.len + 1);
    if (use_tbl) for (int q = lane; q <= sp.len; q += 64) tblm[q] = 0u;
    wsync();
    bool bad = false;
    {
        int4 nxt4 = lane < sp.n_pt ? sp.W.pt[lane] : make_int4(0, 0, 0, 0);
        for (int q = lane; q < sp.n_pt; q += 64) {
            const int4 rec4 = nxt4;
            if (q + 64 < sp.n_pt) nxt4 = sp.W.pt[q + 64];
            const int key = trk_key[rec4.x];
            if (pe_lds) pE[q] = __hiloint2double(rec4.w, rec4.z);
            pkb[q] = ((uint32_t)rec4.y & 0x1ffffu) | ((key < 0 ? 0x7fffu : (uint32_t)key) << 17);
            if (use_tbl && key >= 0) {
                const int d = (int)((uint32_t)rec4.y >> 17);
                if (d >= sp.len) bad = true;
                else {
                    const int row = (q < sp.stale_p1 && sp.stale_d >= 0) ? sp.len : d;
                    tbl[row * n_part + (key >> 2)] = (uint16_t)(q + 1);
                    atomicOr(&tblm[row], 1u << (key >> 2));
                }
            }
        }
    }
    wsync();
    if (WSA_TUNE(DBG_CYCLES)) sp.ph[0] = __builtin_readcyclecounter();
    if (files_past_the_end(sp, lane, !use_tbl, [&](int q) __attribute__((always_inline)) { return (pkb[q] >> 17) != 0x7fffu; })) bad = true;
    if (__ballot(bad) != 0ull) { if (lane == 0) { sp.sg[SEG_FLAG] = -1; sp.sg[SEG_NROWS] = 0; } return true; }
    if (use_tbl) {
        const uint32_t stale_m = tblm[sp.len];
        float thr_f;
        { const double t0 = sp.floor_ < 0 ? 0.0 : floor(sp.floor_) + 1.0; thr_f = (float)(t0 > 256.0 ? 256.0 : t0); }
        for (int base = 0; base < ((WSA_TUNE(DBG_NO_STRAIGHTEN)) ? 0 : sp.len); base += 64) {
            const int d = base + lane;
            float* const row = fr + 9 * (d < sp.len ? d : 0);
            if (d < sp.len) {
#pragma unroll
                for (int q = 0; q < 9; q++) row[q] = 0.f;
            }
            float sm = 0.f;
            auto apply = [&](int q) __attribute__((always_inline)) {
                const uint32_t w = pkb[q];
                int l = (int)((w >> 17) & 3u);
                const double E = energy_of(q);
                const float ff = (float)(w & 0xffu), cur = row[3 * l];
                if (cur >= thr_f && cur < ff && l < 2) l++;
                row[3 * l] = ff; row[3 * l + 1] = (float)E; row[3 * l + 2] = (float)((w >> 8) & 0x1ffu);
                sm = (float)((double)sm + E);
            };
            const uint32_t m_main = d < sp.len ? tblm[d] : 0u, m_st = (d < sp.len && d == sp.stale_d) ? stale_m : 0u;
            uint32_t mm = m_main | m_st;
            while (mm) {
                const int r = __ffs((int)mm) - 1; mm &= mm - 1u;
                if ((m_st >> r) & 1u) apply((int)tbl[sp.len * n_part + r] - 1);
                if ((m_main >> r) & 1u) apply((int)tbl[d * n_part + r] - 1);
            }
            if (d < sp.len) smv[d] = sm;
        }
    } else
    straighten_select<int>(p, sp, lane, fr, smv,
        [&](int q) __attribute__((always_inline)) -> int { const uint32_t w = pkb[q]; return (w >> 17) == 0x7fffu ? -1 : (int)(((w >> 19) << 16) | (uint32_t)q); },
        [&](int q, int& l, double& f, double& wd, double& E) __attribute__((always_inline)) {
            const uint32_t w = pkb[q];
            l = (int)((w >> 17) & 3u); f = w & 0xffu; wd = (w >> 8) & 0x1ffu; E = energy_of(q);
        });
    wsync();
    if (WSA_TUNE(DBG_CYCLES)) sp.ph[1] = __builtin_readcyclecounter();
    double* const red = reinterpret_cast<double*>(L.big + off_pt);
    write_rows<true>(p, sp, lane, fr, smv, [&](const float* f, int n, double* x) __attribute__((always_inline)) {
        formant_features_lds(f, n, sp.ctx_max, x, lane, red, !G && n <= 15 && !(p.dbg & DBG_NO_PACKED_COLUMNS), G || (p.dbg & DBG_EVENTS_BLOCK) != 0);
    });
    return true;
}
template <int AC>
__device__ __forceinline__ void finalize_generic(const TrParams& p, SpanState& sp, const OneLds<AC>& L, int lane) {
    constexpr int FRCAP = OneLds<AC>::FRCAP;
    if (WSA_TUNE(DBG_CYCLES)) sp.ph[0] = sp.ph[1] = sp.ph[2] = sp.ph[3] = __builtin_readcyclecounter();
    const int nq = qualify_tracks(sp.W, sp.n_tr, lane, sp.W.q_mb, sp.W.q_idx, [&](int t) __attribute__((always_inline)) { sp.W.tr_slot[t] = -1; });
    wsync();
    const bool q_lds = nq <= AC;
    double* qmb = sp.W.q_mb; int32_t* qidx = sp.W.q_idx; int32_t* sorted = sp.W.sorted;
    if (q_lds) {
        for (int qi = lane; qi < nq; qi += 64) { L.f_qmb[qi] = sp.W.q_mb[qi]; L.f_qidx[qi] = sp.W.q_idx[qi]; }
        qmb = L.f_qmb; qidx = L.f_qidx; sorted = L.f_sorted;
        wsync();
    }
    rank_tracks(nq, qmb, lane, [&](int rank, int qi) __attribute__((always_inline)) { sorted[rank] = qi; });
    wsync();
    assign_slots(nq, qmb, qidx, sorted, lane, [&](int t, int key) __attribute__((always_inline)) { sp.W.tr_slot[t] = key; });
    wsync();
    {
        int t_nxt = lane < sp.n_pt ? sp.W.pt[lane].x : 0;
        for (int q = lane; q < sp.n_pt; q += 64) {
            const int t = t_nxt;
            if (q + 64 < sp.n_pt) t_nxt = sp.W.pt[q + 64].x;
            sp.W.pt_key[q] = sp.W.tr_slot[t];
        }
    }
    wsync();
    if (WSA_TUNE(DBG_CYCLES)) sp.ph[0] = __builtin_readcyclecounter();
    if (__ballot(files_past_the_end(sp, lane, true, [&](int q) __attribute__((always_inline)) { return sp.W.pt_key[q] >= 0; })) != 0ull) { if (lane == 0) { sp.sg[SEG_FLAG] = -1; sp.sg[SEG_NROWS] = 0; } return; }
    float* const fr = sp.len <= FRCAP ? L.f_fr : sp.W.fr;
    float* const smv_ = sp.len <= FRCAP ? L.f_sm : sp.W.sm1;
    auto features = [&](const float* f, int a, double* x) __attribute__((always_inline)) {
        if (sp.len > FRCAP && a <= FEAT_LDS_MAX) formant_features_lds(f, a, sp.ctx_max, x, lane, reinterpret_cast<double*>(L.big), false, true);
        else formant_features_wave(f, a, sp.ctx_max, x, sp.W.Aev, sp.aev_stride, lane);
    };
    straighten_select<long long>(p, sp, lane, fr, smv_,
        [&](int q) __attribute__((always_inline)) -> long long { const int pk = sp.W.pt_key[q]; return pk < 0 ? -1LL : (long long)(pk >> 2) * (long long)(p.pcap + 1) + q; },
        [&](int q, int& l, double& f, double& wd, double& E) __attribute__((always_inline)) {
            l = sp.W.pt_key[q] & 3;
            const int4 rec4 = sp.W.pt[q];
            f = rec4.y & 0xff; wd = (rec4.y >> 8) & 0x1ff; E = __hiloint2double(rec4.w, rec4.z);
        });
    wsync();
    if (WSA_TUNE(DBG_CYCLES)) sp.ph[1] = __builtin_readcyclecounter();
    write_rows<false>(p, sp, lane, fr, smv_, features);
}
__device__ __forceinline__ void export_raw_tracks(const TrParams& p, SpanState& sp, int lane, bool ring) {
    const int nq = qualify_tracks(sp.W, sp.n_tr, lane, sp.W.q_mb, sp.W.q_idx, [](int) __attribute__((always_inline)) {});
    wsync();
    const uint64_t pbase = (uint64_t)sp.foff * MAXC;
    const uint64_t pmask = ring ? (uint64_t)(p.ring_mask + 1u) * MAXC - 1ull : ~0ull;
    const uint64_t poff = (ring ? (uint64_t)((uint32_t)sp.sg[SEG_FBEGIN] & p.ring_mask) : (uint64_t)sp.f_begin) * MAXC;
    const uint64_t pool0 = pbase + poff;
    auto slot = [&](uint64_t q) __attribute__((always_inline)) -> uint64_t { return pbase + ((poff + q) & pmask); };
    rank_tracks(nq, sp.W.q_mb, lane, [&](int rank, int qi) __attribute__((always_inline)) { p.trk_rank[slot((uint64_t)rank)] = sp.W.q_idx[qi]; });
    for (int q = lane; q < sp.n_pt; q += 64) { int4 v = sp.W.pt[q]; v.y &= 0x1ffff; p.trk_pts[2 * slot((uint64_t)q)] = v; p.trk_pts[2 * slot((uint64_t)q) + 1] = sp.W.ptx[q]; }
    if (lane == 0) {
        int32_t* ts = p.trk_seg + ((uint64_t)sp.clip * p.seg_cap + sp.my_seg) * 4;
        ts[0] = (int32_t)(pool0 & 0xffffffffu); ts[1] = sp.n_pt; ts[2] = nq; ts[3] = (int32_t)(pool0 >> 32);
    }
}
template <int AC, bool RAW, bool THIRD>
__device__ __forceinline__ void finish_span(const TrParams& p, SpanState& sp, const OneLds<AC>& L, int lane, bool ring = false) {
    for (int j = lane; j < sp.n_act; j += 64) { const int gi = L.a_gid[j]; sp.W.tr_len[gi] = L.a_len[j]; sp.W.tr_sumE[gi] = L.a_sumE[j]; sp.W.tr_sumEbin[gi] = L.a_sumEbin[j]; }
    wsync();
    if constexpr (RAW) export_raw_tracks(p, sp, lane, ring);
    else if (!(WSA_TUNE(DBG_NO_FINALIZE))) {
        if (!(p.dbg & DBG_GENERIC_FINALIZE)) {
            if (finalize_lds<AC, false>(p, sp, L, lane)) return;
            if constexpr (THIRD) { if (!(p.dbg & DBG_NO_THIRD_FORM) && finalize_lds<AC, true>(p, sp, L, lane)) return; }
        }
        finalize_generic<AC>(p, sp, L, lane);
    }
}
template <int AC>
__device__ __forceinline__ void finalize_from_header(const TrParams& p, SpanState& sp, const OneLds<AC>& L, int lane) {
    const double* hd = p.span_hdr + ((uint64_t)sp.clip * p.seg_cap + (uint32_t)sp.my_seg) * 8;
    const double h0 = hd[0], h1 = hd[1], h2 = hd[2], h3 = hd[3], h4 = hd[4], h5 = hd[5], h6 = hd[6];
    const int flag = (int)h6;
    if (flag == 0) return;
    if (flag & 2) { if (lane == 0) atomicOr(&p.shared[1], 1u); return; }
    const int F = (int)(sp.f_end - sp.f_begin);
    sp.W = carve_ws(p.pool + (uint64_t)(sp.foff + sp.f_begin) * p.pool_bpf, MAXC * F, MAXC * F, F, 0, nullptr);
    sp.aev_stride = F + 2;
    sp.n_tr = (int)h0; sp.n_pt = (int)h1; sp.n_act = 0; sp.stale_d = (int)h2; sp.stale_p1 = (int)h3;
    sp.accG = h4; sp.accL = lane == 0 ? h5 : 0.0;
    sp.gen = 1;
    const unsigned long long tf0 = WSA_TUNE(DBG_CYCLES) ? __builtin_readcyclecounter() : 0ull;
    finish_span<AC, false, true>(p, sp, L, lane);
    if (WSA_TUNE(DBG_CYCLES) && lane == 0 && p.trace) {
        double* tr = p.trace + (uint64_t)atomicAdd(&p.shared[0], 1u) * 12;
        tr[0] = 0; tr[1] = (double)(__builtin_readcyclecounter() - tf0); tr[2] = sp.len; tr[3] = F; tr[4] = sp.n_tr; tr[5] = sp.n_pt; tr[6] = blockIdx.x;
        tr[7] = (double)(sp.ph[0] - tf0); tr[8] = (double)(sp.ph[1] - sp.ph[0]); tr[9] = (double)(sp.ph[2] - sp.ph[1]); tr[10] = (double)(sp.ph[3] - sp.ph[2]);
    }
    if (sp.overflow && lane == 0) atomicOr(&p.shared[1], 1u);
    wsync();
}

}
```

webspeechanalyzer_amd/csrc/wsa_internal.hpp:

```cpp
#pragma once
#include <hip/hip_runtime.h>
#include <stdint.h>
#include <string>
#include <vector>
#include "../../include/wsa.h"

namespace wsa {

struct FePlanHost {
    int win = 0, hop = 0, nfft = 0, n2 = 0, R = 0, kmax = 0, bands = 0, spec_type = 1;
    int three = 0, M = 0;
    std::vector<float> window;
    std::vector<float> tw_n2;
    std::vector<float> tw_m;
    std::vector<float> tw_64;
    std::vector<float> tw_nfft;
    std::vector<int32_t> mel_k0, mel_cnt, mel_off;
    std::vector<float> mel_w;
    std::vector<float> emph;
    float gain = 0;
    std::vector<double> bins_hz;
};
bool build_fe_plan(const wsa_config& cfg, double fs, FePlanHost& out, std::string& err);

struct Tuning {
    int dbg = 0;
    bool no_pair = false, no_split = false, fe_fat = false, peaks_lanes = false;
    bool no_quad = false, quad = false;
    bool no_fuse = false;
    int full_table = -1;
    int tracker_wpc = 0, fin_wpc = 0;
    int fpw = 0;
    int fe_wg_per_cu = 0;
    bool fe_no_queue = false;
    int peaks_wpc = 0;
    int peaks_w = 0;
    int upload_threads = 0;
    int rs_s = 0, rs_j = 0, rs_c = 0;
    bool rs_one_launch = false;
    static Tuning from_env();
};

enum : int {
    DBG_NO_FINALIZE = 1,
    DBG_NO_ACCUMULATE = 2,
    DBG_NO_FEATURES = 4,
    DBG_NO_STRAIGHTEN = 8,
    DBG_CYCLES = 16,
    DBG_NO_ENTRIES = 32,
    DBG_NO_PREFETCH = 64,
    DBG_GENERIC_FINALIZE = 256,
    DBG_PHASES = 512,
    DBG_SMALL_TABLE = 1024,
    DBG_GATE_F64 = 2048,
    DBG_GATE_GENERAL = 4096,
    DBG_UNSORTED_SPANS = 8192,
    DBG_SMALL_GROUP_TABLE = 16384,
    DBG_SELECT_LOOP = 32768,
    DBG_NO_PACKED_COLUMNS = 65536,
    DBG_EVENTS_BLOCK = 131072,
    DBG_NO_THIRD_FORM = 262144,
    DBG_PEAKS_SHIFT = 20,
};
enum : int {
    PK_DBG_NO_EMISSION = 1,
    PK_DBG_NO_STATE_MACHINE = 2,
    PK_DBG_NO_MASK_PASS = 4,
    PK_DBG_NO_STORES = 8,
    PK_DBG_NO_LDS_ATOMIC = 16,
    PK_DBG_NO_GLOBAL_PATH = 32,
};

struct FeParams {
    const float* pcm = nullptr; uint64_t clip_stride = 0;
    const uint32_t* n_frames = nullptr;
    const uint32_t* frame_off = nullptr;
    uint32_t* spec = nullptr;
    int win = 0, hop = 0, kmax = 0, bands = 0, spec_type = 0, frames_per_wave = 0, mel_total = 0, mel_max_taps = 0;
    int mel_max_taps_lo = 0;
    const float* window = nullptr; const float2* tw_n2 = nullptr; const float2* tw_64 = nullptr; const float2* tw_nfft = nullptr;
    const float2* tw_m = nullptr;
    const int32_t* mel_k0 = nullptr; const int32_t* mel_cnt = nullptr; const int32_t* mel_off = nullptr; const float* mel_w = nullptr;
    const float* emph = nullptr; float gain = 0;
    const uint32_t* pcm_off = nullptr;
    int fat = 0, wg_per_cu = 0;
    uint32_t* queue = nullptr; uint32_t chunks_per_clip = 0, n_chunks = 0; int n_cu = 0;
};

constexpr int CAND_CAP = 64;
struct RecPtrs { uint4* hdr = nullptr; uint32_t* amp = nullptr; uint4* ent = nullptr; };
struct PkParams {
    const uint32_t* spec = nullptr; RecPtrs rec; uint32_t frame0 = 0, total_frames = 0; int bands = 0;
    const double* stream_state = nullptr; const uint32_t* n_frames = nullptr; uint32_t step_frames = 0, ring = 0;
    uint32_t* flags = nullptr;
    int dbg = 0;
    int lanes_only = 0, wpc = 0;
    int round_bins = 0;
};

struct GateParams {
    RecPtrs rec;
    const uint32_t* n_frames = nullptr; const uint32_t* frame_off = nullptr; uint32_t clip0 = 0, n_clips = 0;
    int level = 0, max_voiced_bin = 0; double breaker = 0, min_frames = 0; int auto_gate = 0; double ctx_max0 = 0, floor0 = 0;
    int32_t* fr_info = nullptr;
    double* fr_v = nullptr;
    double* fr_fl = nullptr;
    int32_t* seg_i = nullptr; double* seg_d = nullptr; int seg_cap = 0;
    uint32_t* seg_count = nullptr;
    uint32_t* clip_rows = nullptr;
    uint32_t* counters = nullptr;
    uint32_t* shared = nullptr;
    double* trace = nullptr; int dbg = 0;
    uint32_t* span_hist = nullptr; uint2* span_key = nullptr;
    int strided = 1;
    double* state = nullptr;
    const uint32_t* ctl = nullptr;
    uint32_t ring = 0, step_frames = 0;
    int32_t* fr_span = nullptr;
    int prio = 0;
};
enum { GATE_STATE = 16 };
enum { SEG_START = 0, SEG_LEN = 1, SEG_FBEGIN = 2, SEG_FEND = 3, SEG_CCI = 4, SEG_FLAG = 5, SEG_NROWS = 6, SEG_ROW0 = 7 };

struct TrParams {
    RecPtrs rec;
    const uint32_t* frame_off = nullptr;
    int level = 0;
    const int32_t* fr_info = nullptr; const double* fr_v = nullptr; const double* fr_fl = nullptr;
    int32_t* seg_i = nullptr; const double* seg_d = nullptr; int seg_cap = 0;
    const uint32_t* seg_count = nullptr; uint32_t n_clips = 0; const uint32_t* counters = nullptr; uint32_t* shared = nullptr;
    char* ws = nullptr; uint64_t ws_stride = 0; int tcap = 0, pcap = 0, fcap = 0;
    int32_t* row_meta = nullptr; double* row_feat = nullptr; uint32_t row_cap = 0; uint32_t* clip_rows = nullptr;
    double* trace = nullptr;
    int dbg = 0;
    uint32_t ring_mask = 0xffffffffu;
    float* formants = nullptr;
    int32_t* st_state = nullptr; char* st_act = nullptr;
    const int32_t* fr_span = nullptr; const uint32_t* n_frames_step = nullptr; const double* gate_state = nullptr;
    int4* trk_pts = nullptr; int32_t* trk_rank = nullptr; int32_t* trk_seg = nullptr;
    const uint2* order = nullptr;
    float* sums = nullptr;
    uint2* redo = nullptr; uint32_t* redo_count = nullptr;
    int order_cnt = 1;
    char* pool = nullptr; uint32_t pool_bpf = 0; double* span_hdr = nullptr;
    int fin_waves = 0;
    int quad = 0, quad_waves = 0;
};

struct CompactParams {
    uint32_t n_clips = 0; int seg_cap = 0, level = 0;
    const int32_t* seg_i = nullptr; const uint32_t* seg_count = nullptr;
    const int32_t* row_meta_in = nullptr; const double* row_feat_in = nullptr;
    int32_t* seg_out = nullptr; int32_t* row_meta_out = nullptr; double* row_feat_out = nullptr;
    uint32_t* clip_row_off = nullptr; uint32_t* clip_seg_off = nullptr; uint32_t* totals = nullptr;
    int32_t* carry = nullptr;
    const uint32_t* ctl = nullptr;
    const uint32_t* clip_rows = nullptr; const uint32_t* flags = nullptr; uint32_t* host = nullptr; int fused = 0;
    uint32_t* clr_counters = nullptr; uint32_t* clr_hist = nullptr;
};
bool compact_is_fused(const CompactParams& p);
enum { COMPACT_NOTHING = -1, COMPACT_FUSED = 0, COMPACT_SCAN = 1, COMPACT_COUNT_SCAN = 2 };
int compact_path(const CompactParams& p);
enum { CARRY_HIST = 32, CARRY_WORDS = 2 + 2 * CARRY_HIST };

struct UttParams {
    uint32_t n_clips = 0;
    const int32_t* segments = nullptr; const int32_t* row_meta = nullptr;
    const uint32_t* clip_seg_off = nullptr; const uint32_t* clip_row_off = nullptr; const uint32_t* frame_off = nullptr;
    const float* formants = nullptr;
    uint32_t* clip_utt_off = nullptr;
    int32_t* utt_meta = nullptr; double* utt_feat = nullptr;
    uint32_t* totals = nullptr;
    uint32_t* state = nullptr; const int32_t* carry = nullptr; const uint32_t* ctl = nullptr; uint32_t ring_mask = 0xffffffffu;
};
enum { UTT_STATE_WORDS = 288 };

constexpr int RS_TAPS = 32, RS_OFFS = 32;
struct RsParams {
    const float* in; uint64_t stride_in; float* out; uint64_t stride_out;
    const uint32_t* n_in; const uint32_t* n_out;
    int chunks;
    const float* table; double ratio; int span, S, J;
};
void build_resample_table(double fs_in, double fs_out, std::vector<float>& K);
void resample_table_image(const std::vector<float>& K, std::vector<float>& img);
uint64_t resample_length(uint64_t n_in, double fs_in, double fs_out);
int resample_stride(double fs_in, double fs_out);
int resample_span(double ratio, int S, int J);
int resample_outputs_per_lane(int S, double ratio);
void launch_resample(const RsParams& p, uint32_t n_clips, uint64_t max_out, hipStream_t s);
struct RsClass { double ratio; uint32_t table_off; int span, S, J, copy, pad; };
struct RsWork { uint32_t clip, blk; };
struct RsMixedParams {
    const float* in; uint64_t stride_in; float* out; uint64_t stride_out;
    const uint32_t* n_in; const uint32_t* n_out;
    const float* tables; const RsClass* cls; const uint32_t* clip_class; const RsWork* work;
};
struct RsMixedPlan {
    std::vector<float> tables; std::vector<RsClass> cls; std::vector<uint32_t> clip_class; std::vector<RsWork> work;
    std::vector<uint32_t> first, block, lds;
    uint32_t max_block = 64, max_lds = 0, n_work = 0;
};
bool plan_resample_mixed(uint32_t n_clips, const uint32_t* n_out, const double* fs_in, double fs_out, RsMixedPlan& P, std::string& err);
void launch_resample_mixed(const RsMixedParams& p, const RsMixedPlan& P, bool per_class, hipStream_t s);

enum { RS_CTL_NFR = 0, RS_CTL_OFF = 1, RS_CTL_BITS = 2,
       RS_CTL_NIN = 3, RS_CTL_NOUT = 4,
       RS_CTL_DST = 5,
       RS_CTL_SHIFT = 6, RS_CTL_CARRY = 7,
       RS_CTL_Y_LO = 8, RS_CTL_Y_HI = 9,
       RS_CTL_IN0_LO = 10, RS_CTL_IN0_HI = 11,
       RS_CTL_WORDS = 12 };
constexpr int RS_HIST = 48;
struct RsStreamParams {
    float* stage; uint32_t stage_stride;
    float* conv; uint32_t conv_stride;
    const float* in; uint64_t in_stride;
    float* hist;
    const uint32_t* ctl; uint32_t n;
    const float* tables; const RsClass* cls; const uint32_t* stream_class;
    uint32_t xcap;
};
void launch_resample_stream(const RsStreamParams& p, hipStream_t s);
size_t resample_stream_lds(uint32_t xcap);
uint64_t resample_ready(uint64_t n_in, double fs_in, double fs_out);
uint32_t resample_step_frames_bound(uint32_t frames_per_step, uint32_t hop, double min_ratio);
uint32_t resample_step_outputs_bound(uint32_t frames_per_step, uint32_t hop, double min_ratio);

void launch_frontend(const FeParams& p, int n_clips, int max_frames, int R, int three, hipStream_t s);
bool fe_supported_R(int R, int three);
size_t fe_lds_required(const FePlanHost& P, bool fat);
const char* fe_choice_name(const FePlanHost& P, bool fat);
void launch_peaks(const PkParams& p, hipStream_t s);
void launch_peaks_mode(const PkParams& p, int mode, hipStream_t s);
void launch_gate(const GateParams& p, hipStream_t s);
void launch_gate_stream(const GateParams& p, hipStream_t s);
void launch_gate_blocks(const GateParams& p, uint32_t blocks, hipStream_t s);
void launch_gate_stream_blocks(const GateParams& p, uint32_t blocks, hipStream_t s);
void launch_stream_prepare(double* state, int32_t* carry, int32_t* tr_state, const uint32_t* ctl, uint32_t n, double ctx_max0, double floor0, hipStream_t s);
void launch_tracker(const TrParams& p, int n_waves, bool full_table, bool pair, hipStream_t s);
enum { SPAN_BUCKETS = 2048 };
void launch_span_order(const TrParams& p, uint32_t* span_hist, const uint2* span_key, uint2* order, uint32_t* counters, hipStream_t s);
void launch_tracker_stream(const TrParams& p, uint32_t n_streams, hipStream_t s);
enum { TR_STATE_WORDS = 16, TR_ACT_MAX = 320, TR_ACT_BYTES = TR_ACT_MAX * 44 };
void launch_compact(const CompactParams& p, hipStream_t s);
void launch_utterance(const UttParams& p, hipStream_t s);

struct CoefParams {
    const int32_t* row_meta = nullptr; double* row_feat = nullptr;
    const uint32_t* frame_off = nullptr; const uint32_t* totals = nullptr;
    const float* formants = nullptr; const float* sums = nullptr;
    double* ws = nullptr; uint32_t total_frames = 0;
    uint32_t ring_mask = 0xffffffffu, scratch_stride = 0;
};
void launch_coeffs(const CoefParams& p, uint32_t rows_cap, hipStream_t s);
size_t tracker_ws_bytes(int tcap, int pcap, int fcap, bool raw_tracks);
size_t tracker_pool_bpf();

}
```

Measured before the change: 780.7 million frames/s.

## Add level-specialized lean finalize kernel with device-side decline and full rerun fallback

Adds a finalize kernel templated on output level 5 or 13 that compiles only the LDS fast path, dropping the generic and third-form fallbacks and the packed-columns variant for level 5. This is meant to cut register pressure and code size in the finalize stage. If any span cannot be handled by the lean path, a device counter records the decline and the host reruns the whole backend with the full kernel, setting it sticky for later runs. The cost is an extra readback word and a possible full backend rerun. Debug accessors for finalize state and span loads are also added.

```diff
diff --git a/webspeechanalyzer_amd/capi.py b/webspeechanalyzer_amd/capi.py
--- a/webspeechanalyzer_amd/capi.py
+++ b/webspeechanalyzer_amd/capi.py
@@ -752,6 +752,20 @@
         self.an._check(self.L.wsa_debug_batch_tiers(self.h, stream, out))
         return dict(flags=int(out[0]), spans=int(out[1]), redo=int(out[2]))
 
+    def finalize_kernels(self):
+        out = (ctypes.c_uint32 * 4)()
+        self.L.wsa_debug_batch_finalize.argtypes = [ctypes.c_void_p, ctypes.c_void_p]
+        self.an._check(self.L.wsa_debug_batch_finalize(self.h, out))
+        return dict(kernel=("none", "full", "lean")[int(out[0])], switches=int(out[1]), declined=int(out[2]), full=bool(out[3]))
+
+    def span_loads(self, stream=0):
+        n = ctypes.c_uint32(0)
+        self.L.wsa_debug_batch_span_loads.argtypes = [ctypes.c_void_p, ctypes.c_void_p, ctypes.c_void_p, ctypes.c_uint32, ctypes.c_void_p]
+        self.an._check(self.L.wsa_debug_batch_span_loads(self.h, stream, None, 0, ctypes.byref(n)))
+        out = np.zeros((max(n.value, 1), 6), np.int32)
+        self.an._check(self.L.wsa_debug_batch_span_loads(self.h, stream, out.ctypes.data, n.value, ctypes.byref(n)))
+        return out[:n.value]
+
     def enable_trace(self, on=True):
         self.an._check(self.L.wsa_batch_enable_trace(self.h, int(on)))
 
diff --git a/webspeechanalyzer_amd/csrc/api.hip b/webspeechanalyzer_amd/csrc/api.hip
--- a/webspeechanalyzer_amd/csrc/api.hip
+++ b/webspeechanalyzer_amd/csrc/api.hip
@@ -18,7 +18,7 @@
     t.no_pair = std::getenv("WSA_NO_PAIR") != nullptr; t.no_split = std::getenv("WSA_NO_SPLIT") != nullptr; t.no_quad = std::getenv("WSA_NO_QUAD") != nullptr; t.quad = std::getenv("WSA_QUAD") != nullptr; t.no_fuse = std::getenv("WSA_NO_FUSE") != nullptr;
     t.fe_fat = std::getenv("WSA_FE_FAT") != nullptr; t.peaks_lanes = std::getenv("WSA_PEAKS_LANES") != nullptr;
     t.full_table = num("WSA_FULL_TABLE", -1);
-    t.tracker_wpc = num("WSA_TRACKER_WPC", 0); t.fin_wpc = num("WSA_FIN_WPC", 0); t.fpw = num("WSA_FPW", 0);
+    t.tracker_wpc = num("WSA_TRACKER_WPC", 0); t.fin_wpc = num("WSA_FIN_WPC", 0); t.fin_full = num("WSA_FIN_FULL", 0) != 0; t.fpw = num("WSA_FPW", 0);
     t.fe_wg_per_cu = num("WSA_FE_WGS", 0); t.fe_no_queue = std::getenv("WSA_FE_NO_QUEUE") != nullptr; t.peaks_wpc = num("WSA_PEAKS_WPC", 0); t.peaks_w = num("WSA_PEAKS_W", 0); t.upload_threads = num("WSA_UPLOAD_THREADS", 0);
     t.rs_s = num("WSA_RS_S", 0); t.rs_j = num("WSA_RS_J", 0); t.rs_c = num("WSA_RS_C", 0); t.rs_one_launch = std::getenv("WSA_RS_ONE_LAUNCH") != nullptr;
     return t;
diff --git a/webspeechanalyzer_amd/csrc/batch_internal.hpp b/webspeechanalyzer_amd/csrc/batch_internal.hpp
--- a/webspeechanalyzer_amd/csrc/batch_internal.hpp
+++ b/webspeechanalyzer_amd/csrc/batch_internal.hpp
@@ -42,6 +42,7 @@
     hipEvent_t ev[5] = {nullptr, nullptr, nullptr, nullptr, nullptr};
     bool timing = true, ran = false, full_table = false;
     uint32_t reruns = 0;
+    bool fin_full = false; int fin_kernel = 0; uint32_t fin_switches = 0, fin_declined = 0;
     uint32_t res_rows = 0, res_segs = 0, res_flags = 0;
     const uint32_t* spec_in_use = nullptr;
     wsa_cls* cls = nullptr;
diff --git a/webspeechanalyzer_amd/csrc/batch_run.hip b/webspeechanalyzer_amd/csrc/batch_run.hip
--- a/webspeechanalyzer_amd/csrc/batch_run.hip
+++ b/webspeechanalyzer_amd/csrc/batch_run.hip
@@ -7,7 +7,7 @@
 namespace wsa {
 __global__ void batch_publish_kernel(const uint32_t* totals, const uint32_t* counters, uint32_t* host) {
     if (threadIdx.x == 0) {
-        host[0] = totals[0]; host[1] = totals[1]; host[2] = counters[1]; host[3] = totals[3];
+        host[0] = totals[0]; host[1] = totals[1]; host[2] = counters[1]; host[3] = totals[3]; host[4] = counters[FIN_DECLINED];
         __threadfence_system();
     }
 }
@@ -46,12 +46,14 @@
     t.pool = b->split ? b->d_pool : nullptr; t.pool_bpf = (uint32_t)b->pool_bpf; t.span_hdr = b->split ? b->d_span_hdr : nullptr;
     if (t.order) launch_span_order(t, b->d_span_hist, b->d_span_key, b->d_order, counters, s);
     if (b->timing) HIP_TRY(ctx, hipEventRecord(b->ev[2], s));
-    launch_tracker(t, b->n_waves, b->full_table, b->pair, s);
+    constexpr int FIN_FORM_DBG = DBG_GENERIC_FINALIZE | DBG_NO_THIRD_FORM | DBG_SELECT_LOOP | DBG_EVENTS_BLOCK;
+    t.fin_lean = !b->fin_full && !b->tune.fin_full && !(dbg & FIN_FORM_DBG) ? 1 : 0;
+    b->fin_kernel = launch_tracker(t, b->n_waves, b->full_table, b->pair, s);
     if (b->timing) HIP_TRY(ctx, hipEventRecord(b->ev[3], s));
     CompactParams cp;
     B.fill(cp, D);
     cp.clip_rows = B.d_clip_rows; cp.flags = B.d_counters + 1; cp.fused = b->tune.no_fuse ? 0 : 1;
-    cp.host = D.tail_kernel ? nullptr : b->h_totals_dev;
+    cp.host = D.tail_kernel ? nullptr : b->h_totals_dev; cp.declined = B.d_counters + FIN_DECLINED;
     b->published = compact_is_fused(cp) && cp.host != nullptr;
     const bool self_clear = b->published && !b->capturing && !b->keep_counters;
     cp.clr_counters = self_clear ? B.d_counters : nullptr; cp.clr_hist = self_clear ? b->d_span_hist : nullptr;
@@ -139,6 +141,17 @@
         HIP_TRY(ctx, hipStreamSynchronize(s));
         b->res_rows = ht[0]; b->res_segs = ht[1]; b->res_flags = ht[2]; b->res_utt = ht[3];
     }
+    if (const uint32_t declined = ht[4]; declined != 0u) {
+        b->fin_full = true; b->fin_switches++; b->fin_declined = declined;
+        hipLaunchKernelGGL(batch_clear_kernel, dim3(1), dim3(256), 0, s, b->be.d_counters, b->be.d_totals, b->d_span_hist);
+        const bool tm = b->timing; b->timing = false;
+        const wsa_status st = run_backend_stages(b, b->spec_in_use, true, s);
+        b->timing = tm;
+        if (st != WSA_OK) return st;
+        if (!b->published) hipLaunchKernelGGL(batch_publish_kernel, dim3(1), dim3(64), 0, s, b->be.d_totals, b->be.d_counters, b->h_totals_dev);
+        HIP_TRY(ctx, hipStreamSynchronize(s));
+        b->res_rows = ht[0]; b->res_segs = ht[1]; b->res_flags = ht[2]; b->res_utt = ht[3];
+    }
     if (b->res_flags & 1u) return fail(ctx, WSA_ERR_CAPACITY, "a device-side arena overflowed; results are invalid");
     return WSA_OK;
 }
@@ -177,4 +190,33 @@
     return hipMemcpy(out16, b->be.d_counters, 16 * sizeof(uint32_t), hipMemcpyDeviceToHost) == hipSuccess ? WSA_OK : WSA_ERR_HIP;
 }
 
-}
+int wsa_debug_batch_finalize(wsa_batch* b, uint32_t* out4) {
+    if (!b || !out4) return WSA_ERR_INVALID;
+    out4[0] = (uint32_t)b->fin_kernel; out4[1] = b->fin_switches; out4[2] = b->fin_declined; out4[3] = b->fin_full || b->tune.fin_full ? 1u : 0u;
+    return WSA_OK;
+}
+
+int wsa_debug_batch_span_loads(wsa_batch* b, void* stream, int32_t* out, uint32_t cap, uint32_t* n) {
+    if (!b || !n || (cap && !out)) return WSA_ERR_INVALID;
+    if (!b->split || !b->ran) return WSA_ERR_INVALID;
+    const BackEnd& B = b->be;
+    const size_t slots = (size_t)b->n_clips * (size_t)B.seg_cap;
+    std::vector<uint32_t> cnt(b->n_clips); std::vector<int32_t> seg(slots * 8); std::vector<double> hdr(slots * 8);
+    if (hipSetDevice(b->ctx->device) != hipSuccess) return WSA_ERR_NO_DEVICE;
+    if (hipStreamSynchronize(reinterpret_cast<hipStream_t>(stream)) != hipSuccess
+        || hipMemcpy(cnt.data(), B.d_seg_count, cnt.size() * sizeof(uint32_t), hipMemcpyDeviceToHost) != hipSuccess
+        || hipMemcpy(seg.data(), B.d_seg_i, seg.size() * sizeof(int32_t), hipMemcpyDeviceToHost) != hipSuccess
+        || hipMemcpy(hdr.data(), b->d_span_hdr, hdr.size() * sizeof(double), hipMemcpyDeviceToHost) != hipSuccess) return WSA_ERR_HIP;
+    uint32_t k = 0;
+    for (uint32_t c = 0; c < b->n_clips; c++)
+        for (uint32_t g = 0; g < cnt[c] && g < (uint32_t)B.seg_cap; g++, k++) {
+            if (k >= cap) continue;
+            const size_t e = ((size_t)c * (size_t)B.seg_cap + g) * 8;
+            int32_t* o = out + (size_t)k * 6;
+            o[0] = (int32_t)c; o[1] = (int32_t)g; o[2] = seg[e + SEG_LEN]; o[3] = (int32_t)hdr[e]; o[4] = (int32_t)hdr[e + 1]; o[5] = (int32_t)hdr[e + 6];
+        }
+    *n = k;
+    return WSA_OK;
+}
+
+}
diff --git a/webspeechanalyzer_amd/csrc/tracker.hip b/webspeechanalyzer_amd/csrc/tracker.hip
--- a/webspeechanalyzer_amd/csrc/tracker.hip
+++ b/webspeechanalyzer_amd/csrc/tracker.hip
@@ -225,7 +225,7 @@
         track_group<AC, GW, SPLIT>(p, sp, L, lane, t);
     }
 }
-template <int AC>
+template <int AC, int LV = LV_ANY>
 __device__ __forceinline__ void finalize_body(const TrParams& p) {
     const OneLds<AC> L = carve_lds<AC>();
     const int lane = threadIdx.x;
@@ -235,7 +235,7 @@
     for (;;) {
         if (next_span<DEAL_FINALIZE>(p, t) == SPAN_DONE) break;
         sp.begin(p, t.clip, (int)t.seg); sp.load_segment(p, true);
-        finalize_from_header<AC>(p, sp, L, lane);
+        finalize_from_header<AC, LV>(p, sp, L, lane);
     }
 }
 
@@ -255,6 +255,11 @@
 __global__ __launch_bounds__(64) __attribute__((amdgpu_waves_per_eu(4, 4))) void tracker_kernel_finalize(TrParams p) {
     __builtin_amdgcn_s_setprio(3);
     finalize_body<AC_FAST>(p);
+}
+template <int LV>
+__global__ __launch_bounds__(64) __attribute__((amdgpu_waves_per_eu(4, 4))) void tracker_kernel_finalize_rows(TrParams p) {
+    __builtin_amdgcn_s_setprio(3);
+    finalize_body<AC_FAST, LV>(p);
 }
 __global__ __launch_bounds__(64) void tracker_kernel_full(TrParams p) { one_span_body<AC_MAX, false>(p); }
 __global__ __launch_bounds__(64) void tracker_kernel_raw(TrParams p) { one_span_body<AC_MAX, true>(p); }
@@ -303,15 +308,20 @@
     else hipLaunchKernelGGL(tracker_kernel_stream, dim3(n_streams), dim3(64), 0, s, p);
 }
 
-void launch_tracker(const TrParams& p, int n_waves, bool full_table, bool pair, hipStream_t s) {
-    if (n_waves <= 0) return;
+int launch_tracker(const TrParams& p, int n_waves, bool full_table, bool pair, hipStream_t s) {
+    int fin = FIN_NONE;
+    if (n_waves <= 0) return fin;
     if (p.level == 3) hipLaunchKernelGGL(tracker_kernel_raw, dim3(n_waves), dim3(64), 0, s, p);
     else if (full_table) hipLaunchKernelGGL(tracker_kernel_full, dim3(n_waves), dim3(64), 0, s, p);
     else if (pair && p.order && p.redo && (!p.trace || (p.dbg & DBG_CYCLES))) {
         if (p.pool && p.span_hdr) {
             if (p.quad) hipLaunchKernelGGL(tracker_kernel_quad_acc, dim3(p.quad_waves > 0 ? p.quad_waves : n_waves), dim3(64), 0, s, p);
             else hipLaunchKernelGGL(tracker_kernel_pair_acc, dim3(n_waves), dim3(64), 0, s, p);
-            hipLaunchKernelGGL(tracker_kernel_finalize, dim3(p.fin_waves > 0 ? p.fin_waves : 2 * n_waves), dim3(64), 0, s, p);
+            const dim3 fin_grid(p.fin_waves > 0 ? p.fin_waves : 2 * n_waves);
+            fin = p.fin_lean && (p.level == 5 || p.level == 13) ? FIN_LEAN_KERNEL : FIN_FULL_KERNEL;
+            if (fin == FIN_LEAN_KERNEL && p.level == 5) hipLaunchKernelGGL(tracker_kernel_finalize_rows<5>, fin_grid, dim3(64), 0, s, p);
+            else if (fin == FIN_LEAN_KERNEL) hipLaunchKernelGGL(tracker_kernel_finalize_rows<13>, fin_grid, dim3(64), 0, s, p);
+            else hipLaunchKernelGGL(tracker_kernel_finalize, fin_grid, dim3(64), 0, s, p);
         }
         else hipLaunchKernelGGL(tracker_kernel_pair, dim3(n_waves), dim3(64), 0, s, p);
         TrParams r = p; r.order = p.redo; r.order_cnt = 2; r.pool = nullptr; r.span_hdr = nullptr;
@@ -319,6 +329,7 @@
         hipLaunchKernelGGL(tracker_kernel_fast, dim3(n_waves < redo_waves ? n_waves : redo_waves), dim3(64), 0, s, r);
     }
     else hipLaunchKernelGGL(tracker_kernel_fast, dim3(n_waves), dim3(64), 0, s, p);
+    return fin;
 }
 
 __global__ void compact_count_kernel(CompactParams p) {
@@ -383,7 +394,7 @@
             rt = wave_sum_u32(rt); st = wave_sum_u32(st);
             if (lane == 0) {
                 p.totals[0] = rt; p.totals[1] = st; p.clip_row_off[p.n_clips] = rt; p.clip_seg_off[p.n_clips] = st;
-                if (p.host) { p.host[0] = rt; p.host[1] = st; p.host[2] = p.flags[0]; p.host[3] = p.totals[3]; __threadfence_system(); }
+                if (p.host) { p.host[0] = rt; p.host[1] = st; p.host[2] = p.flags[0]; p.host[3] = p.totals[3]; if (p.declined) p.host[4] = p.declined[0]; __threadfence_system(); }
             }
             if (p.clr_counters) {
                 wsync();
diff --git a/webspeechanalyzer_amd/csrc/tracker_finalize.hpp b/webspeechanalyzer_amd/csrc/tracker_finalize.hpp
--- a/webspeechanalyzer_amd/csrc/tracker_finalize.hpp
+++ b/webspeechanalyzer_amd/csrc/tracker_finalize.hpp
@@ -116,21 +116,24 @@
         }
     }
 }
-template <bool LANES, typename Feat>
+constexpr int LV_ANY = 0;
+template <bool LANES, int LV, typename Feat>
 __device__ __forceinline__ void write_rows(const TrParams& p, SpanState& sp, int lane, const float* fr, const float* smv, Feat&& features) {
-    if (p.formants && (p.level == 4 || p.level == 10)) {
+    static_assert(LV == LV_ANY || LV == 5 || LV == 13, "the levels a kernel is compiled for write feature rows only");
+    const int level = LV == LV_ANY ? p.level : LV;
+    if (p.formants && (level == 4 || level == 10)) {
         for (int q = lane; q < 9 * sp.len; q += 64) { const int d = q / 9; p.formants[((uint64_t)sp.foff + (((uint32_t)sp.start + (uint32_t)d) & p.ring_mask)) * 9 + (uint32_t)(q - 9 * d)] = fr[q]; }
         if (p.sums) { for (int q = lane; q < sp.len; q += 64) p.sums[(uint64_t)sp.foff + (((uint32_t)sp.start + (uint32_t)q) & p.ring_mask)] = smv[q]; }
     }
     double accS, accC; sp.totals(accS, accC);
     const double cs = accC / accS;
     const double lg_ctx = jsm::log10(sp.ctx_max);
-    if (p.level == 4 || p.level == 5) {
+    if (level == 4 || level == 5) {
         const long long r0 = take_rows(p, sp, lane, 1);
         if (r0 < 0) return;
         double* x = p.row_feat + (uint64_t)r0 * WSA_NFEAT;
         if (WSA_TUNE(DBG_CYCLES)) sp.ph[2] = __builtin_readcyclecounter();
-        if (p.level == 5) {
+        if (level == 5) {
             if (!(WSA_TUNE(DBG_NO_FEATURES))) features(fr, sp.len, x);
             if (WSA_TUNE(DBG_CYCLES)) sp.ph[3] = __builtin_readcyclecounter();
             if (lane == 0) { x[0] = sp.len; x[1] = sqrt((double)sp.len); x[2] = cs; x[3] = lg_ctx; x[4] = sp.floor_; }
@@ -171,7 +174,7 @@
     for (int k = 0; k < nsyl; k++) {
         const int si = LANES && k < 64 ? read_lane_i32(my_si, k) : sp.W.q_idx[2 * k], sl = LANES && k < 64 ? read_lane_i32(my_sl, k) : sp.W.q_idx[2 * k + 1];
         double* x = p.row_feat + (uint64_t)(r0 + k) * WSA_NFEAT;
-        if (p.level == 13) {
+        if (level == 13) {
             if (!(WSA_TUNE(DBG_NO_FEATURES))) features(fr + 9 * si, sl, x);
             if (lane == 0) { x[0] = sl; x[1] = sqrt((double)sl); x[2] = cs; x[3] = lg_ctx; x[4] = sp.floor_; }
         } else if (lane < WSA_NFEAT) x[lane] = 0;
@@ -182,7 +185,7 @@
     }
     if (lane == 0) { sp.sg[SEG_FLAG] = nsyl > 0 ? 1 : 0; sp.sg[SEG_NROWS] = nsyl; sp.sg[SEG_ROW0] = (int32_t)r0; }
 }
-template <int AC, bool G>
+template <int AC, bool G, int LV = LV_ANY>
 __device__ __forceinline__ bool finalize_lds(const TrParams& p, SpanState& sp, const OneLds<AC>& L, int lane) {
     constexpr int BIG = OneLds<AC>::BYTES;
     const int off_u = (int)align16((size_t)2 * sp.n_tr);
@@ -278,8 +281,8 @@
     wsync();
     if (WSA_TUNE(DBG_CYCLES)) sp.ph[1] = __builtin_readcyclecounter();
     double* const red = reinterpret_cast<double*>(L.big + off_pt);
-    write_rows<true>(p, sp, lane, fr, smv, [&](const float* f, int n, double* x) __attribute__((always_inline)) {
-        formant_features_lds(f, n, sp.ctx_max, x, lane, red, !G && n <= 15 && !(p.dbg & DBG_NO_PACKED_COLUMNS), G || (p.dbg & DBG_EVENTS_BLOCK) != 0);
+    write_rows<true, LV>(p, sp, lane, fr, smv, [&](const float* f, int n, double* x) __attribute__((always_inline)) {
+        formant_features_lds(f, n, sp.ctx_max, x, lane, red, LV != 5 && !G && n <= 15 && !(p.dbg & DBG_NO_PACKED_COLUMNS), G || (p.dbg & DBG_EVENTS_BLOCK) != 0);
     });
     return true;
 }
@@ -326,7 +329,7 @@
         });
     wsync();
     if (WSA_TUNE(DBG_CYCLES)) sp.ph[1] = __builtin_readcyclecounter();
-    write_rows<false>(p, sp, lane, fr, smv_, features);
+    write_rows<false, LV_ANY>(p, sp, lane, fr, smv_, features);
 }
 __device__ __forceinline__ void export_raw_tracks(const TrParams& p, SpanState& sp, int lane, bool ring) {
     const int nq = qualify_tracks(sp.W, sp.n_tr, lane, sp.W.q_mb, sp.W.q_idx, [](int) __attribute__((always_inline)) {});
@@ -343,20 +346,22 @@
         ts[0] = (int32_t)(pool0 & 0xffffffffu); ts[1] = sp.n_pt; ts[2] = nq; ts[3] = (int32_t)(pool0 >> 32);
     }
 }
-template <int AC, bool RAW, bool THIRD>
-__device__ __forceinline__ void finish_span(const TrParams& p, SpanState& sp, const OneLds<AC>& L, int lane, bool ring = false) {
+template <int AC, bool RAW, bool THIRD, int LV = LV_ANY>
+__device__ __forceinline__ bool finish_span(const TrParams& p, SpanState& sp, const OneLds<AC>& L, int lane, bool ring = false) {
     for (int j = lane; j < sp.n_act; j += 64) { const int gi = L.a_gid[j]; sp.W.tr_len[gi] = L.a_len[j]; sp.W.tr_sumE[gi] = L.a_sumE[j]; sp.W.tr_sumEbin[gi] = L.a_sumEbin[j]; }
     wsync();
     if constexpr (RAW) export_raw_tracks(p, sp, lane, ring);
+    else if constexpr (LV != LV_ANY) { if (!(WSA_TUNE(DBG_NO_FINALIZE))) return finalize_lds<AC, false, LV>(p, sp, L, lane); }
     else if (!(WSA_TUNE(DBG_NO_FINALIZE))) {
         if (!(p.dbg & DBG_GENERIC_FINALIZE)) {
-            if (finalize_lds<AC, false>(p, sp, L, lane)) return;
-            if constexpr (THIRD) { if (!(p.dbg & DBG_NO_THIRD_FORM) && finalize_lds<AC, true>(p, sp, L, lane)) return; }
+            if (finalize_lds<AC, false>(p, sp, L, lane)) return true;
+            if constexpr (THIRD) { if (!(p.dbg & DBG_NO_THIRD_FORM) && finalize_lds<AC, true>(p, sp, L, lane)) return true; }
         }
         finalize_generic<AC>(p, sp, L, lane);
     }
-}
-template <int AC>
+    return true;
+}
+template <int AC, int LV = LV_ANY>
 __device__ __forceinline__ void finalize_from_header(const TrParams& p, SpanState& sp, const OneLds<AC>& L, int lane) {
     const double* hd = p.span_hdr + ((uint64_t)sp.clip * p.seg_cap + (uint32_t)sp.my_seg) * 8;
     const double h0 = hd[0], h1 = hd[1], h2 = hd[2], h3 = hd[3], h4 = hd[4], h5 = hd[5], h6 = hd[6];
@@ -370,7 +375,8 @@
     sp.accG = h4; sp.accL = lane == 0 ? h5 : 0.0;
     sp.gen = 1;
     const unsigned long long tf0 = WSA_TUNE(DBG_CYCLES) ? __builtin_readcyclecounter() : 0ull;
-    finish_span<AC, false, true>(p, sp, L, lane);
+    const bool taken = finish_span<AC, false, LV == LV_ANY, LV>(p, sp, L, lane);
+    if (LV != LV_ANY && !taken) { if (lane == 0) atomicAdd(&p.shared[FIN_DECLINED], 1u); return; }
     if (WSA_TUNE(DBG_CYCLES) && lane == 0 && p.trace) {
         double* tr = p.trace + (uint64_t)atomicAdd(&p.shared[0], 1u) * 12;
         tr[0] = 0; tr[1] = (double)(__builtin_readcyclecounter() - tf0); tr[2] = sp.len; tr[3] = F; tr[4] = sp.n_tr; tr[5] = sp.n_pt; tr[6] = blockIdx.x;
diff --git a/webspeechanalyzer_amd/csrc/wsa_internal.hpp b/webspeechanalyzer_amd/csrc/wsa_internal.hpp
--- a/webspeechanalyzer_amd/csrc/wsa_internal.hpp
+++ b/webspeechanalyzer_amd/csrc/wsa_internal.hpp
@@ -30,6 +30,7 @@
     bool no_fuse = false;
     int full_table = -1;
     int tracker_wpc = 0, fin_wpc = 0;
+    bool fin_full = false;
     int fpw = 0;
     int fe_wg_per_cu = 0;
     bool fe_no_queue = false;
@@ -120,6 +121,7 @@
     int prio = 0;
 };
 enum { GATE_STATE = 16 };
+enum { FIN_DECLINED = 12 };
 enum { SEG_START = 0, SEG_LEN = 1, SEG_FBEGIN = 2, SEG_FEND = 3, SEG_CCI = 4, SEG_FLAG = 5, SEG_NROWS = 6, SEG_ROW0 = 7 };
 
 struct TrParams {
@@ -144,6 +146,7 @@
     int order_cnt = 1;
     char* pool = nullptr; uint32_t pool_bpf = 0; double* span_hdr = nullptr;
     int fin_waves = 0;
+    int fin_lean = 0;
     int quad = 0, quad_waves = 0;
 };
 
@@ -156,6 +159,7 @@
     int32_t* carry = nullptr;
     const uint32_t* ctl = nullptr;
     const uint32_t* clip_rows = nullptr; const uint32_t* flags = nullptr; uint32_t* host = nullptr; int fused = 0;
+    const uint32_t* declined = nullptr;
     uint32_t* clr_counters = nullptr; uint32_t* clr_hist = nullptr;
 };
 bool compact_is_fused(const CompactParams& p);
@@ -238,7 +242,8 @@
 void launch_gate_blocks(const GateParams& p, uint32_t blocks, hipStream_t s);
 void launch_gate_stream_blocks(const GateParams& p, uint32_t blocks, hipStream_t s);
 void launch_stream_prepare(double* state, int32_t* carry, int32_t* tr_state, const uint32_t* ctl, uint32_t n, double ctx_max0, double floor0, hipStream_t s);
-void launch_tracker(const TrParams& p, int n_waves, bool full_table, bool pair, hipStream_t s);
+enum { FIN_NONE = 0, FIN_FULL_KERNEL = 1, FIN_LEAN_KERNEL = 2 };
+int launch_tracker(const TrParams& p, int n_waves, bool full_table, bool pair, hipStream_t s);
 enum { SPAN_BUCKETS = 2048 };
 void launch_span_order(const TrParams& p, uint32_t* span_hist, const uint2* span_key, uint2* order, uint32_t* counters, hipStream_t s);
 void launch_tracker_stream(const TrParams& p, uint32_t n_streams, hipStream_t s);
```

New measurement: 783.7 million frames/s (median of 6 runs). Within noise of the previous version (+0.4%).
